# stdstu12/YUME

Measured on AMD Instinct MI355X. Metric: denoise-steps/sec (Yume-5B 720P, 33-frame latent), higher is better.
Workload: dtype bf16; 1 GPU; Yume-5B-720P random-init, 33-frame 704x1280 clip (latent 48x13x44x80, FramePack lfz=8, L=9460), ODE Euler steps of a 50-step shift-7 schedule, no CFG, one chain per GPU; num_layers=30, parallelism=dp1 (independent chains, replicated weights)

## Files before the change

include/yume_hip.h:

```cpp
#ifndef YUME_HIP_H
#define YUME_HIP_H

#include <stdint.h>

#ifdef __cplusplus
extern "C" {
#endif

#define YUME_OK 0
#define YUME_EINVAL (-1)
#define YUME_ELAUNCH (-2)
#define YUME_EUNSUP (-3)

const char* yume_last_error(void);
#define YUME_ABI_VERSION 9
int yume_abi_version(void);
const char* yume_target_arch(void);

int64_t yume_counter_workspace_bytes(void);
int yume_counter_workspace_init(void* ptr, int64_t bytes, void* stream);

int yume_calibrate_mfma(int64_t iters, int64_t workgroups, void* ticks, void* sink, void* stream);

int yume_adaln_modulate(const float* x, int64_t ldx, int64_t T, int64_t C, float eps,
                        const float* mul, const float* add, int64_t tab_stride,
                        const int32_t* row_idx, int add_one,
                        void* out, int64_t ldo, int out_kind, void* stream);

enum {
    YUME_EPI_BF16 = 0,
    YUME_EPI_BF16_GELU = 1,
    YUME_EPI_F32 = 2,
    YUME_EPI_RESID = 3,
    YUME_EPI_BF16_SPLITT = 4,
    YUME_EPI_BF16_GELU_ERF = 5,
    YUME_EPI_BF16_GEGLU = 6
};
int yume_gemm_bf16(const void* A, int64_t lda, const void* W, int64_t ldw, const float* bias,
                   int64_t M, int64_t N, int64_t K, int epi,
                   void* out, int64_t ldo,
                   const float* gate, int64_t gate_stride, const int32_t* row_idx,
                   void* outT, int64_t ldt, int64_t n_split,
                   int variant, void* stream);

int64_t yume_gemm_workspace_bytes(void);
int yume_gemm_bf16_ws(const void* A, int64_t lda, const void* W, int64_t ldw, const float* bias,
                      int64_t M, int64_t N, int64_t K, int epi,
                      void* out, int64_t ldo,
                      const float* gate, int64_t gate_stride, const int32_t* row_idx,
                      void* outT, int64_t ldt, int64_t n_split,
                      int variant, void* workspace, int64_t workspace_bytes, void* stream);

int yume_rmsnorm_rope(void* buf, int64_t ld, int64_t T, int64_t C, int nparts,
                      const float* w, float eps, const float* rope, int64_t D, void* stream);
int yume_rmsnorm_rows_periodic(void* buf, int64_t ld, int64_t T, int64_t C, const float* w, int64_t wperiod, float eps,
                               void* stream);

#define YUME_ATTN_Q_PRESCALED 0x100
#define YUME_ATTN_KV_PADDED 0x200
int yume_attn_fwd(const void* Q, int64_t ldq, const void* K, int64_t ldk, const void* Vt, int64_t ldvt,
                  void* O, int64_t ldo, int64_t Lq, int64_t Lk, int64_t H, float scale,
                  int accumulate, int variant, void* stream);
int64_t yume_attn_workspace_bytes(int64_t Lq, int64_t Lk, int64_t H);
int yume_attn_fwd_ws(const void* Q, int64_t ldq, const void* K, int64_t ldk, const void* Vt, int64_t ldvt,
                     void* O, int64_t ldo, int64_t Lq, int64_t Lk, int64_t H, float scale,
                     int accumulate, int variant, void* workspace, int64_t workspace_bytes, void* stream);
int yume_attn_fwd_kw(const void* Q, int64_t ldq, const void* K, int64_t ldk, const void* Vt, int64_t ldvt,
                     void* O, int64_t ldo, int64_t Lq, int64_t Lk, int64_t H, float scale,
                     int accumulate, int variant, void* workspace, int64_t workspace_bytes, float last_key_weight, void* stream);
int yume_attn_fwd_seg(const void* Q, int64_t ldq, const void* const* K, int64_t ldk, const void* const* Vt, int64_t ldvt,
                      void* O, int64_t ldo, int64_t nseg, int64_t Lq_seg, int64_t seg_pitch, const int64_t* Lk, int64_t H,
                      float scale, int accumulate, int variant, const float* last_key_weight, void* stream);
int64_t yume_attn_batch_workspace_bytes(int64_t nseg, int64_t Lq_seg, int64_t Lk_seg, int64_t H);
int yume_attn_fwd_batch(const void* Q, int64_t ldq, const void* K, int64_t ldk, const void* Vt, int64_t ldvt,
                        void* O, int64_t ldo, int64_t nseg, int64_t Lq_seg, int64_t q_pitch,
                        int64_t Lk_seg, int64_t k_pitch, int64_t H, float scale, int accumulate, int variant,
                        void* workspace, int64_t workspace_bytes, void* stream);

int yume_linear_smallm_f32(const float* in, int64_t R, int64_t K, const void* W, int w_bf16,
                           const float* bias, int64_t N, int in_act, int out_act,
                           const float* add_table, float* out, void* stream);

int yume_sinusoidal_embed(const double* t, const int32_t* t_index, int64_t R, int64_t dim,
                          float* out, void* stream);

int yume_modulation_table(const float* tab, const float* e0, int64_t B, int64_t R, int64_t W,
                          float* out, void* stream);

int yume_patch_gather(const void* x, int in_bf16, int64_t Cin, int64_t F, int64_t H, int64_t W,
                      int64_t f0, int64_t nf, int64_t kh, int64_t kw,
                      void* out, int64_t Kp, void* stream);

int yume_unpatchify(const float* in, int64_t ldi, int64_t Fr, int64_t Hp, int64_t Wp,
                    int64_t ph, int64_t pw, int64_t Cout, float* out, void* stream);

int yume_cast_bf16(const float* in, int64_t ldi, int64_t rows_valid, int64_t rows, int64_t cols,
                   void* out, int64_t ldo, void* stream);
int yume_transpose_bf16(const void* in, int in_bf16, int64_t ldi, int64_t rows, int64_t cols,
                        void* out, int64_t ldo, void* stream);


enum { YUME_CONV_EPI_ADD = 16, YUME_CONV_EPI_TSPLIT = 17, YUME_CONV_EPI_RMS_SILU = 18 };
int yume_conv3d_cl(const void* x, const void* cache, int64_t ldc, int64_t Tin, int64_t Hin, int64_t Win, int64_t Cin,
                   const void* W, int64_t ldw, const float* bias, int64_t Cout,
                   int kt, int kh, int kw, int st, int sh, int sw, int pt, int ph, int pw, int ups,
                   int64_t To, int64_t Ho, int64_t Wo, int epi, void* out, int64_t ldo,
                   const void* add, int64_t ldadd, const void* zero_page, void* stream);

int yume_vae_rmsnorm_silu(const void* x, int64_t ldx, int64_t M, int64_t C, const float* gamma, const float* beta,
                          int silu, void* y, int64_t ldy, void* stream);

int yume_vae_dupup_add(const void* x, int64_t ldx, int64_t Tin, int64_t Hin, int64_t Win, int64_t Cin,
                       void* y, int64_t ldy, int64_t To, int64_t Cout, int ft, int fs, int toff, void* stream);

int yume_vae_avgdown_add(const void* x, int64_t ldx, int64_t Tin, int64_t Hin, int64_t Win, int64_t Cin,
                         void* y, int64_t ldy, int64_t Cout, int ft, int fs, void* stream);

int yume_softmax_rows(const float* S, int64_t lds, int64_t R, int64_t n, float scale, void* P, int64_t ldp, void* stream);

int yume_vae_pack_input(const void* x, int in_bf16, int64_t C, int64_t T, int64_t H, int64_t W, int ps,
                        const float* mul, const float* add, void* out, int64_t Cpad, void* stream);
int yume_vae_unpack_output(const void* x, int64_t ldx, int64_t T, int64_t H, int64_t W, int64_t Cv, int ps,
                           const float* sub, const float* mul, float lo, float hi, float* out, void* stream);

int yume_frames_u8(const float* video, int64_t C, int64_t T, int64_t H, int64_t W, void* out, void* stream);
int yume_frames_u8_trunc(const float* video, int64_t C, int64_t T, int64_t H, int64_t W, void* out, void* stream);

int yume_rmsnorm_f32(const float* x, int64_t ldx, int64_t T, int64_t C, float eps, const float* w, void* out, int64_t ldo,
                     void* stream);
int yume_gemm_bf16_batched(const void* A, int64_t lda, int64_t strideA, const void* W, int64_t ldw, int64_t strideW,
                           int64_t M, int64_t N, int64_t K, int epi, void* out, int64_t ldo, int64_t strideO,
                           int64_t batch, int variant, void* stream);
int yume_softmax_bias_rows(const float* S, int64_t lds, int64_t strideS, int64_t H, int64_t n, const float* bias,
                           int64_t ldb, void* P, int64_t ldp, int64_t strideP, void* stream);
int64_t yume_gemm_splitk_workspace_bytes(int64_t M, int64_t N, int splits);
int yume_gemm_bf16_splitk(const void* A, int64_t lda, const void* W, int64_t ldw, const float* bias, int64_t M, int64_t N,
                          int64_t K, int epi, void* out, int64_t ldo, int splits, void* workspace, void* stream);

#ifdef __cplusplus
}
#endif
#endif
```

yume_amd/_lib.py:

```python
import ctypes
import os
from ctypes import c_void_p, c_int, c_int64, c_float, c_char_p

_HERE = os.path.dirname(os.path.abspath(__file__))
LIB_PATH = os.environ.get("YUME_HIP_LIB") or os.path.join(_HERE, "lib", "libyume_hip.so")

_P, _I, _L, _F = c_void_p, c_int, c_int64, c_float

SIGNATURES = {
    "yume_last_error": [],
    "yume_abi_version": [],
    "yume_target_arch": [],
    "yume_counter_workspace_bytes": [],
    "yume_counter_workspace_init": [_P, _L, _P],
    "yume_calibrate_mfma": [_L, _L, _P, _P, _P],
    "yume_adaln_modulate": [_P, _L, _L, _L, _F, _P, _P, _L, _P, _I, _P, _L, _I, _P],
    "yume_gemm_bf16": [_P, _L, _P, _L, _P, _L, _L, _L, _I, _P, _L, _P, _L, _P, _P, _L, _L, _I, _P],
    "yume_gemm_workspace_bytes": [],
    "yume_gemm_bf16_ws": [_P, _L, _P, _L, _P, _L, _L, _L, _I, _P, _L, _P, _L, _P, _P, _L, _L, _I, _P, _L, _P],
    "yume_rmsnorm_f32": [_P, _L, _L, _L, _F, _P, _P, _L, _P],
    "yume_gemm_bf16_batched": [_P, _L, _L, _P, _L, _L, _L, _L, _L, _I, _P, _L, _L, _L, _I, _P],
    "yume_gemm_splitk_workspace_bytes": [_L, _L, _I],
    "yume_gemm_bf16_splitk": [_P, _L, _P, _L, _P, _L, _L, _L, _I, _P, _L, _I, _P, _P],
    "yume_softmax_bias_rows": [_P, _L, _L, _L, _L, _P, _L, _P, _L, _L, _P],
    "yume_rmsnorm_rows_periodic": [_P, _L, _L, _L, _P, _L, _F, _P],
    "yume_rmsnorm_rope": [_P, _L, _L, _L, _I, _P, _F, _P, _L, _P],
    "yume_attn_fwd": [_P, _L, _P, _L, _P, _L, _P, _L, _L, _L, _L, _F, _I, _I, _P],
    "yume_attn_workspace_bytes": [_L, _L, _L],
    "yume_attn_fwd_ws": [_P, _L, _P, _L, _P, _L, _P, _L, _L, _L, _L, _F, _I, _I, _P, _L, _P],
    "yume_attn_fwd_kw": [_P, _L, _P, _L, _P, _L, _P, _L, _L, _L, _L, _F, _I, _I, _P, _L, _F, _P],
    "yume_attn_fwd_seg": [_P, _L, _P, _L, _P, _L, _P, _L, _L, _L, _L, _P, _L, _F, _I, _I, _P, _P],
    "yume_attn_batch_workspace_bytes": [_L, _L, _L, _L],
    "yume_attn_fwd_batch": [_P, _L, _P, _L, _P, _L, _P, _L, _L, _L, _L, _L, _L, _L, _F, _I, _I, _P, _L, _P],
    "yume_linear_smallm_f32": [_P, _L, _L, _P, _I, _P, _L, _I, _I, _P, _P, _P],
    "yume_sinusoidal_embed": [_P, _P, _L, _L, _P, _P],
    "yume_modulation_table": [_P, _P, _L, _L, _L, _P, _P],
    "yume_patch_gather": [_P, _I, _L, _L, _L, _L, _L, _L, _L, _L, _P, _L, _P],
    "yume_unpatchify": [_P, _L, _L, _L, _L, _L, _L, _L, _P, _P],
    "yume_cast_bf16": [_P, _L, _L, _L, _L, _P, _L, _P],
    "yume_transpose_bf16": [_P, _I, _L, _L, _L, _P, _L, _P],
    "yume_conv3d_cl": [_P, _P, _L, _L, _L, _L, _L, _P, _L, _P, _L, _I, _I, _I, _I, _I, _I, _I, _I, _I, _I, _L, _L, _L, _I, _P, _L,
                       _P, _L, _P, _P],
    "yume_vae_rmsnorm_silu": [_P, _L, _L, _L, _P, _P, _I, _P, _L, _P],
    "yume_vae_dupup_add": [_P, _L, _L, _L, _L, _L, _P, _L, _L, _L, _I, _I, _I, _P],
    "yume_vae_avgdown_add": [_P, _L, _L, _L, _L, _L, _P, _L, _L, _I, _I, _P],
    "yume_softmax_rows": [_P, _L, _L, _L, _F, _P, _L, _P],
    "yume_vae_pack_input": [_P, _I, _L, _L, _L, _L, _I, _P, _P, _P, _L, _P],
    "yume_frames_u8": [_P, _L, _L, _L, _L, _P, _P],
    "yume_frames_u8_trunc": [_P, _L, _L, _L, _L, _P, _P],
    "yume_vae_unpack_output": [_P, _L, _L, _L, _L, _L, _I, _P, _P, _F, _F, _P, _P],
}
_RES = {"yume_last_error": c_char_p, "yume_target_arch": c_char_p, "yume_gemm_splitk_workspace_bytes": c_int64, "yume_attn_workspace_bytes": c_int64,
        "yume_attn_batch_workspace_bytes": c_int64,
        "yume_counter_workspace_bytes": c_int64, "yume_gemm_workspace_bytes": c_int64}

_lib = None
ABI_VERSION = 9


def load():
    global _lib
    if _lib is not None:
        return _lib
    if not os.path.exists(LIB_PATH):
        raise RuntimeError(
            f"{LIB_PATH} is missing: the HIP extension has not been built. "
            "Run `python -c 'import __graft_entry__ as g; g.build()'` (or `python -m yume_amd.build`). "
            "There is no CPU/PyTorch fallback for the yume_amd hot path.")
    import torch
    lib = ctypes.CDLL(LIB_PATH)
    for name, argtypes in SIGNATURES.items():
        fn = getattr(lib, name)
        fn.argtypes = argtypes
        fn.restype = _RES.get(name, c_int)
    got, arch = int(lib.yume_abi_version()), lib.yume_target_arch()
    if got != ABI_VERSION or arch != b"gfx950":
        raise RuntimeError(f"{LIB_PATH} has ABI version {got} for {arch!r}, this binding needs {ABI_VERSION} for gfx950: "
                           "rebuild with `python -m yume_amd.build --force`")
    _lib = lib
    return lib


def check(rc, what):
    if rc != 0:
        msg = load().yume_last_error()
        raise RuntimeError(f"{what} failed (rc={rc}): {msg.decode() if msg else '?'}")
```

yume_amd/csrc/gemm_bf16.hip:

```cpp
#include "gemm_core.hpp"
#include "gemm_w4.hpp"

using namespace gemm_core;

namespace {
bool w4_auto() {
    static const bool on = [] { const char* v = getenv("YUME_GEMM_W4"); return !v || atoi(v) != 0; }();
    return on;
}
bool gemm_log() {
    static const bool on = [] { const char* v = getenv("YUME_GEMM_LOG"); return v && atoi(v) != 0; }();
    return on;
}
void gemm_log_line(const char* kernel, int64_t M, int64_t N, int64_t K, int epi, int variant, int64_t lda, int64_t ldw, int64_t ldo, int64_t ldt,
                   int64_t n_split, bool ws, int64_t batch) {
    fprintf(stderr, "[gemm_bf16] %s M=%lld N=%lld K=%lld epi=%d variant=%d lda=%lld ldw=%lld ldo=%lld ldt=%lld n_split=%lld ws=%d batch=%lld\n", kernel,
            (long long)M, (long long)N, (long long)K, epi, variant, (long long)lda, (long long)ldw, (long long)ldo, (long long)ldt, (long long)n_split,
            ws ? 1 : 0, (long long)batch);
}
}

extern "C" int64_t yume_gemm_workspace_bytes(void) { return gemm_w4::sk_workspace_bytes(gemm_w4::SK_MAX_SLOTS); }

extern "C" int yume_gemm_bf16(const void* A, int64_t lda, const void* W, int64_t ldw, const float* bias, int64_t M,
                              int64_t N, int64_t K, int epi, void* out, int64_t ldo, const float* gate,
                              int64_t gate_stride, const int32_t* row_idx, void* outT, int64_t ldt, int64_t n_split,
                              int variant, void* stream) {
    return yume_gemm_bf16_ws(A, lda, W, ldw, bias, M, N, K, epi, out, ldo, gate, gate_stride, row_idx, outT, ldt, n_split, variant, nullptr, 0, stream);
}

extern "C" int yume_gemm_bf16_ws(const void* A, int64_t lda, const void* W, int64_t ldw, const float* bias, int64_t M,
                                 int64_t N, int64_t K, int epi, void* out, int64_t ldo, const float* gate,
                                 int64_t gate_stride, const int32_t* row_idx, void* outT, int64_t ldt, int64_t n_split,
                                 int variant, void* workspace, int64_t workspace_bytes, void* stream) {
    YUME_REQUIRE(A && W && out, "gemm_bf16: NULL pointer");
    YUME_REQUIRE(M > 0 && N > 0 && K > 0, "gemm_bf16: empty problem M=%lld N=%lld K=%lld", (long long)M, (long long)N, (long long)K);
    YUME_REQUIRE(M < (1ll << 31) && N < (1ll << 31) && K < (1ll << 31), "gemm_bf16: dimension too large");
    YUME_REQUIRE((K % BK) == 0, "gemm_bf16: K=%lld must be a multiple of %d", (long long)K, BK);
    YUME_REQUIRE((N % 4) == 0, "gemm_bf16: N=%lld must be a multiple of 4", (long long)N);
    YUME_REQUIRE((lda % 8) == 0 && (ldw % 8) == 0, "gemm_bf16: lda/ldw must be multiples of 8 (16-byte rows)");
    YUME_REQUIRE((ldo % 4) == 0, "gemm_bf16: ldo must be a multiple of 4");
    YUME_REQUIRE(((uintptr_t)A % 16) == 0 && ((uintptr_t)W % 16) == 0 && ((uintptr_t)out % 16) == 0, "gemm_bf16: pointers must be 16-byte aligned");
    Problem p;
    p.W = (const unsigned short*)W; p.ldw = ldw;
    p.M = (int)M; p.N = (int)N; p.K = (int)K;
    p.tiles_m = (int)((M + BM - 1) / BM);
    p.tiles_n = (int)((N + BN - 1) / BN);
    p.group_m = 8;
    p.bsW = 0; p.bsO = 0;
    bool sk = false;
    if (variant == 0 && workspace != nullptr && w4_auto() && epi != YUME_EPI_BF16_GEGLU &&
        use_256(p, 0, epi != YUME_EPI_BF16_SPLITT || (n_split % 256) == 0) && gemm_w4::w4_applies(p, lda, epi) &&
        (epi != YUME_EPI_BF16_SPLITT || (ldt % 8) == 0)) {
        Problem q = p;
        q.tiles_m = (int)((M + 255) / 256);
        q.tiles_n = (int)((N + 255) / 256);
        gemm_w4::w4_sk_plan(q, workspace, workspace_bytes);
        sk = q.sk_wgs != 0;
    }
    if (!sk && variant == 0 && epi != YUME_EPI_BF16_GEGLU && use_256(p, 0, epi != YUME_EPI_BF16_SPLITT || (n_split % 256) == 0)) {
        const int64_t tn = (N + 255) / 256, tm = (M + 255) / 256, T = tm * tn, R = T % 256, full = T - R;
        const int64_t m_main = full / tn, M_main = m_main * 256, rem = M - M_main;
        if (R > 0 && R <= 96 && full >= 256 && m_main >= 1 && rem > 0 && rem <= 1024) {
            const int64_t osz = (epi == YUME_EPI_F32 || epi == YUME_EPI_RESID) ? 4 : 2;
            auto remainder = [&](void* s2) {
                return yume_gemm_bf16(reinterpret_cast<const unsigned short*>(A) + M_main * lda, lda, W, ldw, bias, rem, N, K, epi,
                                      reinterpret_cast<char*>(out) + M_main * ldo * osz, ldo, gate, gate_stride,
                                      row_idx ? row_idx + M_main : nullptr,
                                      outT ? reinterpret_cast<unsigned short*>(outT) + M_main : nullptr, ldt, n_split, 1, s2);
            };
            int rc = yume_gemm_bf16(A, lda, W, ldw, bias, M_main, N, K, epi, out, ldo, gate, gate_stride, row_idx, outT, ldt, n_split,
                                    w4_auto() ? 3 : 2, stream);
            if (rc != YUME_OK) return rc;
            return remainder(stream);
        }
    }
    PlainA al;
    al.A = (const unsigned short*)A; al.lda = lda; al.M = (int)M; al.bsA = 0;
    Epilogue e = {};
    e.bias = bias;
    e.out = out; e.ldo = ldo;
    e.gate = gate; e.gate_stride = gate_stride; e.row_idx = row_idx;
    e.outT = (unsigned short*)outT; e.ldt = ldt; e.n_split = (int)n_split;
    hipStream_t st = (hipStream_t)stream;
    const bool split_ok = epi != YUME_EPI_BF16_SPLITT || (n_split % 256) == 0;
    const bool big = use_256(p, variant == 3 ? 2 : variant, split_ok);
    const bool w4 = (variant == 3 || (variant == 0 && big && w4_auto())) && split_ok && gemm_w4::w4_applies(p, lda, epi) &&
                    (epi != YUME_EPI_BF16_SPLITT || (ldt % 8) == 0);
    if (gemm_log())
        gemm_log_line(epi == YUME_EPI_BF16_GEGLU ? "g256" : w4 ? (sk ? "w4+sk" : "w4") : big ? "g256" : "g128", M, N, K, epi, variant, lda, ldw, ldo, ldt,
                      n_split, workspace != nullptr, 1);
#define YUME_GO(E) (w4 ? gemm_w4::launch_w4(E, p, al, e, st, "gemm_bf16", variant == 0 ? workspace : nullptr, workspace_bytes) : big ? launch256<E>(p, al, e, st, "gemm_bf16") : launch<E>(p, al, e, st, "gemm_bf16"))
    switch (epi) {
        case YUME_EPI_BF16: return YUME_GO(YUME_EPI_BF16);
        case YUME_EPI_BF16_GELU: return YUME_GO(YUME_EPI_BF16_GELU);
        case YUME_EPI_BF16_GELU_ERF: return YUME_GO(YUME_EPI_BF16_GELU_ERF);
        case YUME_EPI_F32: return YUME_GO(YUME_EPI_F32);
        case YUME_EPI_RESID:
            YUME_REQUIRE(gate == nullptr || (gate_stride % 4) == 0, "gemm_bf16: gate_stride must be a multiple of 4");
            return YUME_GO(YUME_EPI_RESID);
        case YUME_EPI_BF16_GEGLU:
            YUME_REQUIRE((N % 8) == 0 && bias == nullptr, "gemm_bf16: GEGLU needs N %% 8 == 0 and no bias");
            return launch256<YUME_EPI_BF16_GEGLU>(p, al, e, st, "gemm_bf16");
        case YUME_EPI_BF16_SPLITT:
            YUME_REQUIRE(outT != nullptr && n_split >= 0 && (n_split % BN) == 0 && ldt >= M && (ldt % 4) == 0,
                         "gemm_bf16: SPLITT needs outT, n_split %% 128 == 0, ldt >= M and ldt %% 4 == 0");
            YUME_REQUIRE(((uintptr_t)outT % 16) == 0, "gemm_bf16: outT must be 16-byte aligned");
            return YUME_GO(YUME_EPI_BF16_SPLITT);
        default:
            yume_set_error("gemm_bf16: unknown epilogue %d", epi);
            return YUME_EINVAL;
    }
}

extern "C" int yume_gemm_bf16_batched(const void* A, int64_t lda, int64_t strideA, const void* W, int64_t ldw, int64_t strideW,
                                      int64_t M, int64_t N, int64_t K, int epi, void* out, int64_t ldo, int64_t strideO,
                                      int64_t batch, int variant, void* stream) {
    (void)variant;
    YUME_REQUIRE(A && W && out, "gemm_bf16_batched: NULL pointer");
    YUME_REQUIRE(epi == YUME_EPI_BF16 || epi == YUME_EPI_F32, "gemm_bf16_batched: only the plain bf16 / fp32 epilogues");
    YUME_REQUIRE(batch >= 1 && batch <= 65535, "gemm_bf16_batched: batch %lld", (long long)batch);
    YUME_REQUIRE(M > 0 && N > 0 && K > 0 && M < (1ll << 31) && N < (1ll << 31) && K < (1ll << 31), "gemm_bf16_batched: bad problem size");
    YUME_REQUIRE((K % BK) == 0 && (N % 4) == 0, "gemm_bf16_batched: K must be a multiple of %d and N of 4", BK);
    YUME_REQUIRE((lda % 8) == 0 && (ldw % 8) == 0 && (ldo % 4) == 0, "gemm_bf16_batched: lda/ldw must be multiples of 8, ldo of 4");
    YUME_REQUIRE((strideA % 8) == 0 && (strideW % 8) == 0 && (strideO % 8) == 0, "gemm_bf16_batched: strides must keep 16-byte alignment");
    YUME_REQUIRE(((uintptr_t)A % 16) == 0 && ((uintptr_t)W % 16) == 0 && ((uintptr_t)out % 16) == 0, "gemm_bf16_batched: pointers must be 16-byte aligned");
    Problem p;
    p.W = (const unsigned short*)W; p.ldw = ldw;
    p.M = (int)M; p.N = (int)N; p.K = (int)K;
    p.tiles_m = (int)((M + BM - 1) / BM);
    p.tiles_n = (int)((N + BN - 1) / BN);
    p.group_m = 8;
    p.bsW = strideW;
    p.bsO = strideO * (epi == YUME_EPI_F32 ? 4 : 2);
    PlainA al;
    al.A = (const unsigned short*)A; al.lda = lda; al.M = (int)M; al.bsA = strideA;
    Epilogue e = {};
    e.out = out; e.ldo = ldo;
    hipStream_t st = (hipStream_t)stream;
    if (gemm_log()) gemm_log_line("batched", M, N, K, epi, variant, lda, ldw, ldo, 0, 0, false, batch);
    if (epi == YUME_EPI_F32) return launch<YUME_EPI_F32>(p, al, e, st, "gemm_bf16_batched", (int)batch);
    return launch<YUME_EPI_BF16>(p, al, e, st, "gemm_bf16_batched", (int)batch);
}

namespace {
template <int EPI>
__global__ __launch_bounds__(256) void splitk_reduce_kernel(const float* __restrict__ ws, int splits, int64_t MN, int N,
                                                            const float* __restrict__ bias, void* __restrict__ out, int64_t ldo) {
    const int64_t nq = MN >> 2;
    for (int64_t i = (int64_t)blockIdx.x * blockDim.x + threadIdx.x; i < nq; i += (int64_t)gridDim.x * blockDim.x) {
        f32x4 v = *reinterpret_cast<const f32x4*>(ws + 4 * i);
        for (int s = 1; s < splits; ++s) v += *reinterpret_cast<const f32x4*>(ws + s * MN + 4 * i);
        const int64_t m = (4 * i) / N;
        const int n = (int)((4 * i) - m * N);
        if (bias) v += *reinterpret_cast<const f32x4*>(bias + n);
        if (EPI == YUME_EPI_F32) {
            *reinterpret_cast<f32x4*>(reinterpret_cast<float*>(out) + m * ldo + n) = v;
        } else if (EPI == YUME_EPI_RESID) {
            float* xo = reinterpret_cast<float*>(out) + m * ldo + n;
            *reinterpret_cast<f32x4*>(xo) = *reinterpret_cast<const f32x4*>(xo) + v;
        } else if (EPI == YUME_EPI_BF16_GEGLU) {
            const unsigned o = pack_bf16x2(v[1] * gelu_tanh(v[0]), v[3] * gelu_tanh(v[2]));
            *reinterpret_cast<unsigned*>(reinterpret_cast<unsigned short*>(out) + m * ldo + (n >> 1)) = o;
        } else {
            if (EPI == YUME_EPI_BF16_GELU) {
#pragma unroll
                for (int q = 0; q < 4; ++q) v[q] = gelu_tanh(v[q]);
            }
            if (EPI == YUME_EPI_BF16_GELU_ERF) {
#pragma unroll
                for (int q = 0; q < 4; ++q) v[q] = 0.5f * v[q] * (1.0f + erff(v[q] * 0.7071067811865476f));
            }
            u32x2 o;
            o[0] = pack_bf16x2(v[0], v[1]);
            o[1] = pack_bf16x2(v[2], v[3]);
            *reinterpret_cast<u32x2*>(reinterpret_cast<unsigned short*>(out) + m * ldo + n) = o;
        }
    }
}
}

extern "C" int64_t yume_gemm_splitk_workspace_bytes(int64_t M, int64_t N, int splits) { return (int64_t)splits * M * N * 4; }

extern "C" int yume_gemm_bf16_splitk(const void* A, int64_t lda, const void* W, int64_t ldw, const float* bias, int64_t M, int64_t N,
                                     int64_t K, int epi, void* out, int64_t ldo, int splits, void* workspace, void* stream) {
    YUME_REQUIRE(A && W && out && workspace, "gemm_bf16_splitk: NULL pointer");
    YUME_REQUIRE(splits >= 1 && splits <= 64 && (K % (splits * BK)) == 0, "gemm_bf16_splitk: K=%lld must be a multiple of splits*%d (splits=%d)",
                 (long long)K, BK, splits);
    YUME_REQUIRE(M > 0 && N > 0 && (N % 8) == 0 && (ldo % 4) == 0, "gemm_bf16_splitk: N must be a multiple of 8, ldo of 4");
    YUME_REQUIRE(((uintptr_t)workspace % 16) == 0 && ((uintptr_t)out % 16) == 0, "gemm_bf16_splitk: pointers must be 16-byte aligned");
    YUME_REQUIRE((M * N) % 4 == 0, "gemm_bf16_splitk: M*N must be a multiple of 4");
    const int64_t Ks = K / splits;
    int rc = yume_gemm_bf16_batched(A, lda, Ks, W, ldw, Ks, M, N, Ks, YUME_EPI_F32, workspace, N, M * N, splits, 1, stream);
    if (rc != YUME_OK) return rc;
    const int64_t MN = M * N;
    const unsigned grid = (unsigned)((MN / 4 + 255) / 256 > 16384 ? 16384 : (MN / 4 + 255) / 256);
    hipStream_t st = (hipStream_t)stream;
    const float* ws = (const float*)workspace;
    if (gemm_log() && (epi == YUME_EPI_F32 || epi == YUME_EPI_RESID || epi == YUME_EPI_BF16 || epi == YUME_EPI_BF16_GELU || epi == YUME_EPI_BF16_GELU_ERF ||
                       epi == YUME_EPI_BF16_GEGLU))
        gemm_log_line("splitk_reduce", M, N, K, epi, 0, lda, ldw, ldo, 0, 0, true, splits);
#define YUME_RED(E) hipLaunchKernelGGL((splitk_reduce_kernel<E>), dim3(grid), dim3(256), 0, st, ws, splits, MN, (int)N, bias, out, ldo)
    switch (epi) {
        case YUME_EPI_F32: YUME_RED(YUME_EPI_F32); break;
        case YUME_EPI_RESID: YUME_RED(YUME_EPI_RESID); break;
        case YUME_EPI_BF16: YUME_RED(YUME_EPI_BF16); break;
        case YUME_EPI_BF16_GELU: YUME_RED(YUME_EPI_BF16_GELU); break;
        case YUME_EPI_BF16_GELU_ERF: YUME_RED(YUME_EPI_BF16_GELU_ERF); break;
        case YUME_EPI_BF16_GEGLU: YUME_RED(YUME_EPI_BF16_GEGLU); break;
        default:
            yume_set_error("gemm_bf16_splitk: unsupported epilogue %d", epi);
            return YUME_EINVAL;
    }
    YUME_CHECK_LAUNCH("gemm_bf16_splitk");
    return YUME_OK;
}
```

yume_amd/csrc/gemm_w4.hpp:

```cpp
#pragma once
#include "gemm_core.hpp"
#include "trace.hpp"

namespace gemm_w4 {
using namespace gemm_core;

constexpr int NTHR_W4 = 256;
constexpr int OPER_BYTES = 256 * 128;
constexpr int BUF_BYTES = 2 * OPER_BYTES;
constexpr int LDS_W4 = 2 * BUF_BYTES;

#define W4_AG8(n) "a" #n "0", "a" #n "1", "a" #n "2", "a" #n "3", "a" #n "4", "a" #n "5", "a" #n "6", "a" #n "7", "a" #n "8", "a" #n "9"
#define W4_AGPRS "a0", "a1", "a2", "a3", "a4", "a5", "a6", "a7", "a8", "a9", W4_AG8(1), W4_AG8(2), W4_AG8(3), W4_AG8(4), W4_AG8(5), W4_AG8(6), \
    W4_AG8(7), W4_AG8(8), W4_AG8(9), W4_AG8(10), W4_AG8(11), W4_AG8(12), W4_AG8(13), W4_AG8(14), W4_AG8(15), W4_AG8(16), W4_AG8(17), W4_AG8(18), \
    W4_AG8(19), W4_AG8(20), W4_AG8(21), W4_AG8(22), W4_AG8(23), W4_AG8(24), "a250", "a251", "a252", "a253", "a254", "a255"

#define W4_MFMA2(T0, X0, Y0, T1, X1, Y1)                                                                                                         \
    asm volatile("v_mfma_f32_16x16x32_bf16 a[%c4:%c5], %0, %1, a[%c4:%c5]\n\tv_mfma_f32_16x16x32_bf16 a[%c6:%c7], %2, %3, a[%c6:%c7]"             \
                 ::"v"(X0), "v"(Y0), "v"(X1), "v"(Y1), "n"((T0) * 4), "n"((T0) * 4 + 3), "n"((T1) * 4), "n"((T1) * 4 + 3) : "memory", W4_AGPRS)
#define W4_MFMA2_DMA(T0, X0, Y0, T1, X1, Y1, voff, sbase, lbase, loff)                                                                            \
    asm volatile("s_add_u32 m0, %10, %11\n\tv_mfma_f32_16x16x32_bf16 a[%c4:%c5], %0, %1, a[%c4:%c5]\n\tglobal_load_lds_dwordx4 %8, %9\n\t"         \
                 "v_mfma_f32_16x16x32_bf16 a[%c6:%c7], %2, %3, a[%c6:%c7]"                                                                       \
                 ::"v"(X0), "v"(Y0), "v"(X1), "v"(Y1), "n"((T0) * 4), "n"((T0) * 4 + 3), "n"((T1) * 4), "n"((T1) * 4 + 3), "v"(voff), "s"(sbase),   \
                 "s"(lbase), "n"(loff) : "memory", "scc", W4_AGPRS)
#define W4_MFMA2_DMAB(T0, X0, Y0, T1, X1, Y1, voff, srd, soff, lbase, loff)                                                                           \
    asm volatile("s_add_u32 m0, %11, %12\n\tv_mfma_f32_16x16x32_bf16 a[%c4:%c5], %0, %1, a[%c4:%c5]\n\tbuffer_load_dwordx4 %8, %9, %10 offen lds\n\t"  \
                 "v_mfma_f32_16x16x32_bf16 a[%c6:%c7], %2, %3, a[%c6:%c7]"                                                                           \
                 ::"v"(X0), "v"(Y0), "v"(X1), "v"(Y1), "n"((T0) * 4), "n"((T0) * 4 + 3), "n"((T1) * 4), "n"((T1) * 4 + 3), "v"(voff), "s"(srd),         \
                 "s"(soff), "s"(lbase), "n"(loff) : "memory", "scc", W4_AGPRS)
#define W4_DMAB(voff, srd, soff, lbase, loff) \
    asm volatile("s_add_u32 m0, %3, %4\n\ts_nop 0\n\tbuffer_load_dwordx4 %0, %1, %2 offen lds" ::"v"(voff), "s"(srd), "s"(soff), "s"(lbase), "n"(loff) : "memory", "scc")
#define W4_DMA(voff, sbase, lbase, loff) \
    asm volatile("s_add_u32 m0, %2, %3\n\ts_nop 0\n\tglobal_load_lds_dwordx4 %0, %1" ::"v"(voff), "s"(sbase), "s"(lbase), "n"(loff) : "memory", "scc")

template <int R>
__device__ __forceinline__ f32x4 acc_tile() {
    f32x4 v;
    asm volatile("v_accvgpr_read_b32 %0, a[%c4]\n\tv_accvgpr_read_b32 %1, a[%c5]\n\tv_accvgpr_read_b32 %2, a[%c6]\n\tv_accvgpr_read_b32 %3, a[%c7]"
                 : "=v"(v[0]), "=v"(v[1]), "=v"(v[2]), "=v"(v[3]) : "n"(R * 4), "n"(R * 4 + 1), "n"(R * 4 + 2), "n"(R * 4 + 3) : W4_AGPRS);
    return v;
}
template <int R>
__device__ __forceinline__ void acc_tile_add(f32x4 d) {
    f32x4 v = acc_tile<R>();
    v += d;
    asm volatile("v_accvgpr_write_b32 a[%c4], %0\n\tv_accvgpr_write_b32 a[%c5], %1\n\tv_accvgpr_write_b32 a[%c6], %2\n\tv_accvgpr_write_b32 a[%c7], %3"
                 ::"v"(v[0]), "v"(v[1]), "v"(v[2]), "v"(v[3]), "n"(R * 4), "n"(R * 4 + 1), "n"(R * 4 + 2), "n"(R * 4 + 3) : W4_AGPRS);
}
template <int R0, int N>
__device__ __forceinline__ void acc_zero() {
    if constexpr (N > 0) {
        asm volatile("v_accvgpr_write_b32 a[%c0], 0\n\tv_accvgpr_write_b32 a[%c1], 0\n\tv_accvgpr_write_b32 a[%c2], 0\n\tv_accvgpr_write_b32 a[%c3], 0"
                     ::"n"(R0), "n"(R0 + 1), "n"(R0 + 2), "n"(R0 + 3) : W4_AGPRS);
        acc_zero<R0 + 4, N - 4>();
    }
}
template <int I0, int N, typename F>
__device__ __forceinline__ void static_for(F&& f) {
    if constexpr (N > 0) {
        f(std::integral_constant<int, I0>{});
        static_for<I0 + 1, N - 1>(f);
    }
}

struct Ctx {
    char* smem;
    bf16x8_t fa[2][8], fb[2][8];
    unsigned ra1, rb1, ra0n, rb0n;
    unsigned va[8], vb[8];
    const char* pa;
    const char* pb;
    unsigned lcur;
    i32x4 srd;
    unsigned soff, tapmask;
    unsigned mask[8];
    unsigned par[8];
    unsigned uh[2], uw[2];
};

__device__ __forceinline__ bf16x8_t w4_frag(const Ctx& c, unsigned off) { return *reinterpret_cast<const bf16x8_t*>(c.smem + off); }

#define W4_PIECE_LOFF(q) (((q) >> 3) * OPER_BYTES + ((q) & 7) * 4096)

#define W4_X(g) (SWAP ? c.fb[(g) >> 6][(g) & 7] : c.fa[(g) >> 6][((g) & 63) >> 3])
#define W4_Y(g) (SWAP ? c.fa[(g) >> 6][((g) & 63) >> 3] : c.fb[(g) >> 6][(g) & 7])
#define W4_PAIR(g) W4_MFMA2((g) & 63, W4_X(g), W4_Y(g), ((g) + 1) & 63, W4_X((g) + 1), W4_Y((g) + 1))
#define W4_PAIR_DMA(g, voff, sbase, loff) \
    W4_MFMA2_DMA((g) & 63, W4_X(g), W4_Y(g), ((g) + 1) & 63, W4_X((g) + 1), W4_Y((g) + 1), voff, sbase, c.lcur, loff)
#define W4_PAIR_DMAB(g, voff, loff) \
    W4_MFMA2_DMAB((g) & 63, W4_X(g), W4_Y(g), ((g) + 1) & 63, W4_X((g) + 1), W4_Y((g) + 1), voff, c.srd, c.soff, c.lcur, loff)

#ifndef W4_PLAN
#define W4_PLAN 1
#endif
#ifndef W4_ABLATE
#define W4_ABLATE 0
#endif
#ifndef W4_BAR_B
#define W4_BAR_B 35
#endif
#ifndef W4_BAR_A
#define W4_BAR_A 17
#endif
#ifndef W4_DMA0
#define W4_DMA0 (W4_BAR_A + 2)
#endif
constexpr int P_BAR_A = W4_BAR_A;
constexpr int P_BAR_B = W4_BAR_B;
constexpr int dma_pos(int q) { return W4_PLAN == 0 ? W4_DMA0 + q : W4_DMA0 + (q * (63 - W4_DMA0)) / 15; }
constexpr int piece_at(int pos) {
    for (int q = 0; q < 16; ++q)
        if (dma_pos(q) == pos) return q;
    return -1;
}
constexpr int pieces_before_bar_b() {
    int k = 0;
    for (int q = 0; q < 16; ++q) k += dma_pos(q) <= P_BAR_B ? 1 : 0;
    return k;
}
constexpr int P_F0_FIRST = P_BAR_B + 2;
static_assert(P_F0_FIRST + 16 <= 64 && dma_pos(15) <= 63 && 15 < P_BAR_A && dma_pos(0) > P_BAR_A, "the plan must fit the 64 slots");

template <int CONV>
__device__ __forceinline__ unsigned w4_conv_voff(const Ctx& c, int q) {
    unsigned v = c.va[q];
    if constexpr (CONV == 2) v += ((c.par[q] & 1u) ? c.uh[1] : c.uh[0]) + ((c.par[q] & 2u) ? c.uw[1] : c.uw[0]);
    return (c.mask[q] & c.tapmask) ? v : 0xffffffffu;
}

template <int g, bool DMA, bool SWAP, int CONV>
__device__ __forceinline__ void w4_gaps(Ctx& c) {
    if constexpr (g < 128) {
        {
            constexpr int k = g >> 1, pos = k;
            constexpr int q = (DMA && !(W4_ABLATE & 1)) ? piece_at(pos) : -1;
            if constexpr (q >= 0 && q < 8) {
                if constexpr (CONV != 0) W4_PAIR_DMAB(g, w4_conv_voff<CONV>(c, q & 7), W4_PIECE_LOFF(q & 15));
                else W4_PAIR_DMA(g, c.va[q & 7], c.pa, W4_PIECE_LOFF(q & 15));
            } else if constexpr (q >= 8) W4_PAIR_DMA(g, c.vb[q & 7], c.pb, W4_PIECE_LOFF(q & 15));
            else W4_PAIR(g);
            if constexpr (pos >= 0 && pos < 16 && !(W4_ABLATE & 2)) {
                if constexpr (pos < 8) c.fb[1][pos & 7] = w4_frag(c, c.rb1 + (pos & 7) * 2048);
                else c.fa[1][pos & 7] = w4_frag(c, c.ra1 + (pos & 7) * 2048);
            }
            if constexpr (k == P_BAR_A) {
                if constexpr ((W4_ABLATE & 20) == 20) asm volatile("" ::: "memory");
                else if constexpr (W4_ABLATE & 16) asm volatile("s_barrier" ::: "memory");
                else if constexpr (W4_ABLATE & 4) asm volatile("s_waitcnt lgkmcnt(0)" ::: "memory");
                else asm volatile("s_waitcnt lgkmcnt(0)\n\ts_barrier" ::: "memory");
            }
            if constexpr (k == P_BAR_B) {
                constexpr int keep = (DMA && !(W4_ABLATE & 1)) ? pieces_before_bar_b() : 0;
                if constexpr ((W4_ABLATE & 12) == 12) asm volatile("" ::: "memory");
                else if constexpr (W4_ABLATE & 8) asm volatile("s_barrier" ::: "memory");
                else if constexpr (W4_ABLATE & 4) asm volatile("s_waitcnt vmcnt(%c0)" ::"n"(keep) : "memory");
                else asm volatile("s_waitcnt vmcnt(%c0)\n\ts_barrier" ::"n"(keep) : "memory");
            }
            if constexpr (pos >= P_F0_FIRST && pos < P_F0_FIRST + 16 && !(W4_ABLATE & 2)) {
                constexpr int r = pos - P_F0_FIRST;
                if constexpr (r < 8) c.fb[0][r & 7] = w4_frag(c, c.rb0n + (r & 7) * 2048);
                else c.fa[0][r & 7] = w4_frag(c, c.ra0n + (r & 7) * 2048);
            }
            w4_gaps<g + 2, DMA, SWAP, CONV>(c);
        }
    }
}
template <int q, int CONV>
__device__ __forceinline__ void w4_stage_all(Ctx& c) {
    if constexpr (q < 16) {
        if constexpr (q < 8) {
            if constexpr (CONV != 0) W4_DMAB(w4_conv_voff<CONV>(c, q & 7), c.srd, c.soff, c.lcur, W4_PIECE_LOFF(q));
            else W4_DMA(c.va[q & 7], c.pa, c.lcur, W4_PIECE_LOFF(q));
        } else W4_DMA(c.vb[q & 7], c.pb, c.lcur, W4_PIECE_LOFF(q));
        w4_stage_all<q + 1, CONV>(c);
    }
}

template <int EPI>
__device__ __forceinline__ f32x4 w4_act(f32x4 v) {
    if (EPI == YUME_EPI_BF16_GELU) {
        const f32x2_t lo = gelu_tanh2(f32x2_t{v[0], v[1]}), hi = gelu_tanh2(f32x2_t{v[2], v[3]});
        v = f32x4{lo[0], lo[1], hi[0], hi[1]};
    }
    if (EPI == YUME_EPI_BF16_GELU_ERF) {
#pragma unroll
        for (int q = 0; q < 4; ++q) v[q] = 0.5f * v[q] * (1.0f + erff(v[q] * 0.7071067811865476f));
    }
    return v;
}

__device__ __forceinline__ void w4_store_image(char* smem, unsigned short* dst, int64_t ld, int row0, int rows_valid, int col0, int cols_valid) {
    const int lane = threadIdx.x & 63;
    const int wave = __builtin_amdgcn_readfirstlane(threadIdx.x >> 6);
    const int l31 = lane & 31, rh = lane >> 5;
    if (cols_valid == 256) {
        const unsigned lrow = (unsigned)((wave * 64 + rh) * 512), lch = (unsigned)((l31 ^ rh) << 4);
        char* o = reinterpret_cast<char*>(dst + col0 + l31 * 8) + (int64_t)(row0 + wave * 64 + rh) * ld * 2;
        const int64_t step = ld * 4;
        const int rleft = rows_valid - wave * 64 - rh;
        auto rows = [&](auto pred) {
            constexpr bool PRED = decltype(pred)::value;
#pragma unroll
            for (int g = 0; g < 4; ++g) {
                u32x4 d[8];
#pragma unroll
                for (int u = 0; u < 8; ++u) {
                    const int it = g * 8 + u;
                    d[u] = *reinterpret_cast<const u32x4*>(smem + lrow + it * 1024 + (lch ^ (unsigned)(32 * (it & 15))));
                }
#pragma unroll
                for (int u = 0; u < 8; ++u) {
                    const int it = g * 8 + u;
                    if (!PRED || 2 * it < rleft) *reinterpret_cast<u32x4*>(o + it * step) = d[u];
                }
            }
        };
        if (rows_valid == 256) rows(std::false_type{});
        else rows(std::true_type{});
        return;
    }
    unsigned short* out = dst + col0 + l31 * 8;
    const int col_left = cols_valid - l31 * 8;
#pragma unroll 2
    for (int it = 0; it < 32; ++it) {
        const int r = wave * 64 + it * 2 + rh;
        const u32x4 d = *reinterpret_cast<const u32x4*>(smem + r * 512 + (((l31 ^ r) & 31) << 4));
        if (r < rows_valid && col_left > 0) {
            unsigned short* o = out + (int64_t)(row0 + r) * ld;
            if (col_left >= 8) {
                *reinterpret_cast<u32x4*>(o) = d;
            } else {
#pragma unroll
                for (int q = 0; q < 7; ++q)
                    if (q < col_left) o[q] = (unsigned short)(d[q >> 1] >> (16 * (q & 1)));
            }
        }
    }
}

struct ImageOff { unsigned e[8], o[8]; };
__device__ __forceinline__ ImageOff w4_image_offsets(int rsel, int csel, int l15, int l4) {
    ImageOff r;
    const unsigned base = (unsigned)((rsel * 128 + l15) * 512 + (l4 & 1) * 8), ux = (unsigned)(((l4 >> 1) ^ l15) << 4);
#pragma unroll
    for (int b = 0; b < 8; ++b) {
        const unsigned ob = (unsigned)(32 * b) ^ ux;
        r.e[b] = base + 256u * (unsigned)csel + ob;
        r.o[b] = base + 256u * (unsigned)(csel ^ 1) + ob;
    }
    return r;
}

template <int EPI, bool SWAP>
__device__ __forceinline__ void w4_epilogue(const Problem& p, const Epilogue& e, int m0, int n0, char* smem) {
    const int lane = threadIdx.x & 63;
    const int wave = __builtin_amdgcn_readfirstlane(threadIdx.x >> 6);
    const int wr = wave >> 1, wc = wave & 1;
    const int l15 = lane & 15, l4 = lane >> 4;
    constexpr bool BF16_OUT = EPI == YUME_EPI_BF16 || EPI == YUME_EPI_BF16_GELU || EPI == YUME_EPI_BF16_GELU_ERF || EPI == YUME_EPI_BF16_SPLITT ||
                              EPI == EPI_BF16_ADD || EPI == EPI_BF16_TSPLIT;
    if constexpr (!SWAP) {
        float bn[8];
#pragma unroll
        for (int j = 0; j < 8; ++j) bn[j] = e.bias ? e.bias[min(n0 + wc * 128 + 16 * j + l15, p.N - 1)] : 0.f;
        const ImageOff io = w4_image_offsets(wc, wr, l15, l4);
        asm volatile("s_waitcnt lgkmcnt(0)\n\ts_barrier" ::: "memory");
        static_for<0, 64>([&](auto tt) {
            constexpr int T = decltype(tt)::value, i = T >> 3, j = T & 7;
            const f32x4 v = acc_tile<T>();
            u32x2 o;
            o[0] = pack_bf16x2(v[0] + bn[j], v[1] + bn[j]);
            o[1] = pack_bf16x2(v[2] + bn[j], v[3] + bn[j]);
            *reinterpret_cast<u32x2*>(smem + ((j & 1) ? io.o[i] : io.e[i]) + j * 8192) = o;
        });
        asm volatile("s_waitcnt lgkmcnt(0)\n\ts_barrier" ::: "memory");
        w4_store_image(smem, e.outT + (int64_t)(n0 - e.n_split) * e.ldt, e.ldt, 0, min(256, p.N - n0), m0, min(256, p.M - m0));
        return;
    } else {
        if (BF16_OUT && !p.epi_direct && (e.ldo % 8) == 0) {
            f32x4 b[8];
            if (n0 + 256 <= p.N) {
#pragma unroll
                for (int j = 0; j < 8; ++j)
                    b[j] = e.bias ? *reinterpret_cast<const f32x4*>(e.bias + n0 + wc * 128 + 16 * j + 4 * l4) : f32x4{0.f, 0.f, 0.f, 0.f};
            } else {
#pragma unroll
                for (int j = 0; j < 8; ++j) {
                    const int n = n0 + wc * 128 + 16 * j + 4 * l4;
                    b[j] = (e.bias && n + 3 < p.N) ? *reinterpret_cast<const f32x4*>(e.bias + n) : f32x4{0.f, 0.f, 0.f, 0.f};
                }
            }
            const ImageOff io = w4_image_offsets(wr, wc, l15, l4);
            asm volatile("s_waitcnt lgkmcnt(0)\n\ts_barrier" ::: "memory");
            TRACE_STAMP(3);
            static_for<0, 8>([&](auto ii) {
                constexpr int i = decltype(ii)::value;
                u32x2 a2[8];
                if constexpr (EPI == EPI_BF16_ADD) {
                    const int r = wr * 128 + 16 * i + l15;
                    const int nl = n0 + wc * 128 + 4 * l4;
                    const unsigned short* ap = e.add + (int64_t)min(m0 + r, p.M - 1) * e.ldadd + nl;
#pragma unroll
                    for (int j = 0; j < 8; ++j)
                        a2[j] = nl + 16 * j + 3 < p.N ? *reinterpret_cast<const u32x2*>(ap + 16 * j) : u32x2{0u, 0u};
                }
                static_for<0, 8>([&](auto jj) {
                    constexpr int j = decltype(jj)::value;
                    f32x4 v = w4_act<EPI>(acc_tile<i * 8 + j>() + b[j]);
                    if constexpr (EPI == EPI_BF16_ADD) {
                        v[0] += bf16_to_f32((unsigned short)(a2[j][0] & 0xffffu));
                        v[1] += bf16_to_f32((unsigned short)(a2[j][0] >> 16));
                        v[2] += bf16_to_f32((unsigned short)(a2[j][1] & 0xffffu));
                        v[3] += bf16_to_f32((unsigned short)(a2[j][1] >> 16));
                    }
                    u32x2 o;
                    o[0] = pack_bf16x2(v[0], v[1]);
                    o[1] = pack_bf16x2(v[2], v[3]);
                    *reinterpret_cast<u32x2*>(smem + ((i & 1) ? io.o[j] : io.e[j]) + i * 8192) = o;
                });
            });
            asm volatile("s_waitcnt lgkmcnt(0)\n\ts_barrier" ::: "memory");
            TRACE_STAMP(4);
            if constexpr (EPI == EPI_BF16_TSPLIT) {
                const int ch = p.N >> 1, jh = n0 >= ch ? 1 : 0, t = m0 / e.hw;
                w4_store_image(smem, reinterpret_cast<unsigned short*>(e.out), e.ldo, m0 + (t + jh) * e.hw, min(256, p.M - m0), n0 - jh * ch, 256);
            } else {
                w4_store_image(smem, reinterpret_cast<unsigned short*>(e.out), e.ldo, m0, min(256, p.M - m0), n0, min(256, p.N - n0));
            }
            return;
        }
        if (EPI == YUME_EPI_RESID && n0 + 256 <= p.N) {
            f32x4 b[8];
#pragma unroll
            for (int j = 0; j < 8; ++j)
                b[j] = e.bias ? *reinterpret_cast<const f32x4*>(e.bias + n0 + wc * 128 + 16 * j + 4 * l4) : f32x4{0.f, 0.f, 0.f, 0.f};
            const int mrow = m0 + wr * 128 + l15, ncol = n0 + wc * 128 + 4 * l4;
            const bool ragged_m = m0 + 256 > p.M;
            const int mlast = p.M - 1 - mrow;
            float* const xo = reinterpret_cast<float*>(e.out) + (int64_t)mrow * e.ldo + ncol;
            const int64_t xstep = 16 * e.ldo;
            auto xoff = [&](int i) -> int64_t { return ragged_m ? (int64_t)(min(16 * i, mlast) ) * e.ldo : i * xstep; };
            const bool gated = e.gate != nullptr;
            bool rowed = gated && e.row_idx != nullptr;
            int ridx[8];
#pragma unroll
            for (int i = 0; i < 8; ++i) ridx[i] = rowed ? e.row_idx[min(mrow + 16 * i, p.M - 1)] : 0;
            f32x4 x[2][8], g[2][8];
            auto issue_x = [&](auto ii, auto bb) {
                constexpr int i = decltype(ii)::value, bf = decltype(bb)::value;
#pragma unroll
                for (int j = 0; j < 8; ++j) x[bf][j] = *reinterpret_cast<const f32x4*>(xo + xoff(i) + 16 * j);
            };
            auto issue_g = [&](auto ii, auto bb) {
                constexpr int i = decltype(ii)::value, bf = decltype(bb)::value;
                if (rowed || (gated && i < 2)) {
                    const float* gp = e.gate + (int64_t)ridx[i] * e.gate_stride + ncol;
#pragma unroll
                    for (int j = 0; j < 8; ++j) g[bf][j] = *reinterpret_cast<const f32x4*>(gp + 16 * j);
                }
            };
            issue_x(std::integral_constant<int, 0>{}, std::integral_constant<int, 0>{});
            issue_x(std::integral_constant<int, 1>{}, std::integral_constant<int, 1>{});
            if (rowed) {
                const int r0 = __builtin_amdgcn_readfirstlane(ridx[0]);
                bool same = true;
#pragma unroll
                for (int i = 0; i < 8; ++i) same &= ridx[i] == r0;
                if (__all(same)) rowed = false;
            }
            issue_g(std::integral_constant<int, 0>{}, std::integral_constant<int, 0>{});
            issue_g(std::integral_constant<int, 1>{}, std::integral_constant<int, 1>{});
            TRACE_STAMP(3);
            static_for<0, 8>([&](auto ii) {
                constexpr int i = decltype(ii)::value, bf = i & 1;
                static_for<0, 8>([&](auto jj) {
                    constexpr int j = decltype(jj)::value;
                    const f32x4 v = acc_tile<i * 8 + j>() + b[j];
                    if (gated) x[bf][j] += v * g[bf][j];
                    else x[bf][j] += v;
                    if (!ragged_m || 16 * i <= mlast) *reinterpret_cast<f32x4*>(xo + i * xstep + 16 * j) = x[bf][j];
                });
                if constexpr (i + 2 < 8) {
                    issue_x(std::integral_constant<int, i + 2>{}, std::integral_constant<int, bf>{});
                    issue_g(std::integral_constant<int, i + 2>{}, std::integral_constant<int, bf>{});
                }
                if (i == 0) TRACE_STAMP(4);
            });
            TRACE_STAMP(5);
#ifdef YUME_TRACE
            asm volatile("s_waitcnt vmcnt(0)" ::: "memory");
            TRACE_STAMP(6);
#endif
            return;
        }
        static_for<0, 64>([&](auto tt) {
            constexpr int T = decltype(tt)::value, i = T >> 3, j = T & 7;
            const f32x4 v = acc_tile<T>();
            const int m = m0 + wr * 128 + 16 * i + l15, n = n0 + wc * 128 + 16 * j + 4 * l4;
            if (m < p.M && n < p.N) store_row4<EPI>(v, m, n, p, e);
        });
    }
}

template <bool DMA, bool SWAP>
__device__ __forceinline__ void w4_loop(Ctx& c, int t0, int t1, unsigned lbase) {
    for (int t = t0; t < t1; ++t) {
        w4_gaps<0, DMA, SWAP, 0>(c);
        if constexpr (DMA) {
            c.pa += 128;
            c.pb += 128;
        }
        c.lcur = lbase + (((t + 1) & 1) ? BUF_BYTES : 0);
        c.ra1 ^= BUF_BYTES;
        c.rb1 ^= BUF_BYTES;
        c.ra0n ^= BUF_BYTES;
        c.rb0n ^= BUF_BYTES;
    }
}

template <bool SWAP>
__device__ __forceinline__ void w4_mainloop(const Problem& p, const PlainA& al, char* smem, int m0, int n0, int kt0, int nk) {
    const int tid = threadIdx.x;
    const int lane = tid & 63;
    const int wave = __builtin_amdgcn_readfirstlane(tid >> 6);
    const int wr = wave >> 1, wc = wave & 1;
    Ctx c;
    c.smem = smem;
    const unsigned lbase = (unsigned)(uintptr_t)(__attribute__((address_space(3))) char*)smem + wave * 1024;
    c.lcur = lbase;
    c.pa = reinterpret_cast<const char*>(al.A + (int64_t)m0 * al.lda) + (int64_t)kt0 * 128;
    c.pb = reinterpret_cast<const char*>(p.W + (int64_t)n0 * p.ldw) + (int64_t)kt0 * 128;
    const unsigned lda_b = (unsigned)al.lda * 2u, ldw_b = (unsigned)p.ldw * 2u;
    {
        const int rl = 8 * wave + (lane >> 3);
        const unsigned ch = (unsigned)(((lane & 7) ^ (rl & 7)) << 4);
        const int mleft = p.M - 1 - m0, nleft = p.N - 1 - n0;
#pragma unroll
        for (int j = 0; j < 8; ++j) {
            const int r = 32 * j + rl;
            c.va[j] = (unsigned)min(r, mleft) * lda_b + ch;
            c.vb[j] = (unsigned)min(r, nleft) * ldw_b + ch;
        }
    }
    const unsigned sw0 = (unsigned)(((lane >> 4) ^ (lane & 7)) << 4), sw1 = (unsigned)(((4 | (lane >> 4)) ^ (lane & 7)) << 4);
    const unsigned rowa = wr * 16384 + (lane & 15) * 128, rowb = OPER_BYTES + wc * 16384 + (lane & 15) * 128;
    w4_stage_all<0, 0>(c);
    c.pa += 128;
    c.pb += 128;
    c.lcur = lbase + BUF_BYTES;
    w4_stage_all<0, 0>(c);
    c.pa += 128;
    c.pb += 128;
    c.lcur = lbase;
    acc_zero<0, 256>();
    asm volatile("s_waitcnt vmcnt(16)\n\ts_barrier" ::: "memory");
#pragma unroll
    for (int r = 0; r < 8; ++r) {
        c.fb[0][r] = w4_frag(c, rowb + sw0 + r * 2048);
        c.fa[0][r] = w4_frag(c, rowa + sw0 + r * 2048);
    }
    c.ra1 = rowa + sw1;
    c.rb1 = rowb + sw1;
    c.ra0n = BUF_BYTES + rowa + sw0;
    c.rb0n = BUF_BYTES + rowb + sw0;
    w4_loop<true, SWAP>(c, 0, nk - 2, lbase);
    w4_loop<false, SWAP>(c, nk - 2, nk, lbase);
    asm volatile("s_waitcnt lgkmcnt(0)\n\ts_barrier" ::: "memory");
    asm volatile("s_nop 15\n\ts_nop 15" ::: "memory");
}

constexpr int SK_SLOT_BYTES = 64 * NTHR_W4 * 16;
constexpr int SK_FLAG_STRIDE = 64;
constexpr int SK_MIN_KT = 4;
constexpr int SK_MAX_SLOTS = 256;
constexpr unsigned SK_SPIN_LIMIT = 1u << 22;

__host__ __device__ __forceinline__ int64_t sk_workspace_bytes(int slots) { return (int64_t)slots * (SK_SLOT_BYTES + SK_FLAG_STRIDE) + 64; }

template <int T0, int N>
__device__ __forceinline__ void sk_publish_tiles(const char* slot, unsigned lane_off) {
    if constexpr (N > 0) {
        const f32x4 v = acc_tile<T0>();
        asm volatile("global_store_dwordx4 %0, %1, %2 sc1\n\ts_nop 1" ::"v"(lane_off + (unsigned)(T0 * (NTHR_W4 * 16))), "v"(v), "s"(slot) : "memory");
        sk_publish_tiles<T0 + 1, N - 1>(slot, lane_off);
    }
}
template <int T0, int N>
__device__ __forceinline__ void sk_gather_tiles(const char* slot, unsigned lane_off) {
    if constexpr (N > 0) {
        f32x4 d[8];
#pragma unroll
        for (int u = 0; u < 8; ++u) d[u] = *reinterpret_cast<const f32x4*>(slot + (lane_off + (unsigned)((T0 + u) * (NTHR_W4 * 16))));
        static_for<0, 8>([&](auto uu) {
            constexpr int u = decltype(uu)::value;
            acc_tile_add<T0 + u>(d[u]);
        });
        sk_gather_tiles<T0 + 8, N - 8>(slot, lane_off);
    }
}

template <bool SWAP>
__device__ __forceinline__ void w4_finish_piece(const Problem& p, const Epilogue& e, int epi, char* smem, int m0, int n0, int slot, int t, int nslice) {
    typedef unsigned gu32;
    char* const slots = p.sk_ws;
    gu32* const flags = reinterpret_cast<gu32*>(p.sk_ws + (int64_t)SK_MAX_SLOTS * SK_SLOT_BYTES);
    unsigned lane_off = threadIdx.x * 16u;
    asm volatile("" : "+v"(lane_off));
    if (slot >= 0) {
        sk_publish_tiles<0, 64>(slots + (int64_t)slot * SK_SLOT_BYTES, lane_off);
        asm volatile("s_waitcnt vmcnt(0)" ::: "memory");
        __syncthreads();
        if (threadIdx.x == 0) __hip_atomic_store(flags + slot * (SK_FLAG_STRIDE / 4), 1u, __ATOMIC_RELAXED, __HIP_MEMORY_SCOPE_AGENT);
        return;
    }
    if (nslice > 1) {
        for (int j = 1; j < nslice; ++j) {
            const int q = (j - 1) * p.sk_tiles + t;
            if (threadIdx.x == 0) {
                gu32* f = flags + q * (SK_FLAG_STRIDE / 4);
                unsigned spins = 0;
                while (__hip_atomic_load(f, __ATOMIC_RELAXED, __HIP_MEMORY_SCOPE_AGENT) == 0u) {
                    __builtin_amdgcn_s_sleep(8);
                    if (++spins > SK_SPIN_LIMIT) {
                        __hip_atomic_store(flags + SK_MAX_SLOTS * (SK_FLAG_STRIDE / 4), 1u, __ATOMIC_RELAXED, __HIP_MEMORY_SCOPE_AGENT);
                        break;
                    }
                }
                __builtin_amdgcn_fence(__ATOMIC_ACQUIRE, "agent");
                asm volatile("s_waitcnt vmcnt(0)" ::: "memory");
            }
            __syncthreads();
            sk_gather_tiles<0, 64>(slots + (int64_t)q * SK_SLOT_BYTES, lane_off);
            __syncthreads();
            if (threadIdx.x == 0) __hip_atomic_store(flags + q * (SK_FLAG_STRIDE / 4), 0u, __ATOMIC_RELAXED, __HIP_MEMORY_SCOPE_AGENT);
        }
        asm volatile("s_nop 15" ::: "memory");
    }
    TRACE_STAMP(1);
    if constexpr (!SWAP) {
        w4_epilogue<YUME_EPI_BF16_SPLITT, false>(p, e, m0, n0, smem);
    } else {
        switch (epi) {
#ifndef W4_EXPERIMENT
            case YUME_EPI_BF16_GELU: w4_epilogue<YUME_EPI_BF16_GELU, true>(p, e, m0, n0, smem); break;
            case YUME_EPI_BF16_GELU_ERF: w4_epilogue<YUME_EPI_BF16_GELU_ERF, true>(p, e, m0, n0, smem); break;
            case YUME_EPI_F32: w4_epilogue<YUME_EPI_F32, true>(p, e, m0, n0, smem); break;
            case YUME_EPI_RESID: w4_epilogue<YUME_EPI_RESID, true>(p, e, m0, n0, smem); break;
            case YUME_EPI_BF16_SPLITT: w4_epilogue<YUME_EPI_BF16_SPLITT, true>(p, e, m0, n0, smem); break;
#endif
            default: w4_epilogue<YUME_EPI_BF16, true>(p, e, m0, n0, smem); break;
        }
    }
}

template <int UNUSED = 0>
__global__ __launch_bounds__(NTHR_W4, 1) void gemm_w4_kernel(Problem p, PlainA al, Epilogue e, int epi) {
    __shared__ __attribute__((aligned(16))) char smem[LDS_W4];
    TRACE_STAMP(0);
    const int nk = p.K / BK;
    const int ndp = p.sk_wgs ? p.sk_dp : p.tiles_m * p.tiles_n;
    int pc0 = 0, pc1 = 1, R = 1, tile0, head_t = 0;
    bool tails = false;
    if ((int)blockIdx.x < ndp) {
        int start, count;
        xcd_chunk(ndp, blockIdx.x & 7, start, count);
        tile0 = start + (blockIdx.x >> 3);
    } else {
        const int sk = (int)blockIdx.x - ndp, per = p.sk_wgs >> 3;
        const int w = (sk & 7) * per + (sk >> 3);
        R = p.sk_tiles;
        tile0 = ndp;
        if (w < R) {
            head_t = w;
        } else {
            tails = true;
            const int ntail = (p.sk_s - 1) * R;
            pc0 = (w - R) * p.sk_q;
            pc1 = min(ntail, pc0 + p.sk_q);
            if (pc0 >= pc1) return;
        }
    }
    for (int pc = pc0; pc < pc1; ++pc) {
        int t = head_t, j = 0, k0 = 0, k1 = nk, slot = -1, nslice = 1;
        if (p.sk_wgs && (int)blockIdx.x >= ndp) {
            if (tails) {
                j = 1 + pc / R;
                t = pc - (j - 1) * R;
                k0 = p.sk_lh + (j - 1) * p.sk_lt;
                k1 = j == p.sk_s - 1 ? nk : k0 + p.sk_lt;
                slot = pc;
            } else {
                k1 = p.sk_lh;
                nslice = p.sk_s;
            }
        }
        int m0, n0;
        tile_origin(p, tile0 + t, m0, n0);
        if (epi == YUME_EPI_BF16_SPLITT && n0 >= e.n_split) {
            w4_mainloop<false>(p, al, smem, m0, n0, k0, k1 - k0);
            w4_finish_piece<false>(p, e, epi, smem, m0, n0, slot, t, nslice);
        } else {
            w4_mainloop<true>(p, al, smem, m0, n0, k0, k1 - k0);
            w4_finish_piece<true>(p, e, epi, smem, m0, n0, slot, t, nslice);
        }
        if (pc + 1 < pc1) __syncthreads();
    }
    TRACE_STAMP(2);
}

inline bool w4_applies(const Problem& p, int64_t lda, int epi) {
    if (p.K < 3 * BK) return false;
#ifdef W4_EXPERIMENT
    if (epi != YUME_EPI_BF16) return false;
#endif
    if (255ll * lda * 2 + 128 >= (1ll << 32) || 255ll * p.ldw * 2 + 128 >= (1ll << 32)) return false;
    return epi == YUME_EPI_BF16 || epi == YUME_EPI_BF16_GELU || epi == YUME_EPI_BF16_GELU_ERF || epi == YUME_EPI_F32 || epi == YUME_EPI_RESID ||
           epi == YUME_EPI_BF16_SPLITT;
}

inline void w4_sk_plan(Problem& p, void* ws, int64_t ws_bytes) {
    p.sk_dp = 0; p.sk_tiles = 0; p.sk_wgs = 0; p.sk_s = 1; p.sk_q = 1; p.sk_lh = 0; p.sk_lt = 0; p.sk_ws = nullptr;
    static const bool on = [] { const char* v = getenv("YUME_GEMM_SK"); return !v || atoi(v) != 0; }();
    static const int ncu = [] {
        int d = 0, n = 0;
        if (hipGetDevice(&d) != hipSuccess || hipDeviceGetAttribute(&n, hipDeviceAttributeMultiprocessorCount, d) != hipSuccess) n = 0;
        return n;
    }();
    if (!on || ws == nullptr || ncu < 64 || ncu > SK_MAX_SLOTS || (ncu & 7) != 0) return;
    if (ws_bytes < sk_workspace_bytes(SK_MAX_SLOTS) || ((uintptr_t)ws & 15) != 0) return;
    const int T = p.tiles_m * p.tiles_n, nk = p.K / BK;
    const int R = T % ncu;
    if (R == 0 || T < ncu) return;
    static const int min_nk = [] { const char* v = getenv("YUME_GEMM_SK_MIN_NK"); return v ? atoi(v) : 96; }();
    if (nk < min_nk) return;
    int s, q, lh, lt;
    if (2 * R > ncu) {
        s = 2;
        q = (R + (ncu - R) - 1) / (ncu - R);
        lt = nk / (q + 1);
        lh = nk - lt;
    } else {
        s = ncu / R;
        if (s > nk / SK_MIN_KT) s = nk / SK_MIN_KT;
        q = 1;
        lt = nk / s;
        lh = lt;
    }
    if (s < 2 || lt < SK_MIN_KT || lh < SK_MIN_KT || (s - 1) * R > SK_MAX_SLOTS) return;
    const int nwg = R + ((s - 1) * R + q - 1) / q;
    if (nwg > ncu) return;
    p.sk_tiles = R;
    p.sk_dp = T - R;
    p.sk_s = s; p.sk_q = q; p.sk_lh = lh; p.sk_lt = lt;
    p.sk_wgs = (nwg + 7) / 8 * 8;
    p.sk_ws = (char*)ws;
}

inline int launch_w4(int epi, const Problem& p128, const PlainA& al, const Epilogue& e, hipStream_t st, const char* what, void* ws = nullptr,
                     int64_t ws_bytes = 0) {
    Problem p = p128;
    p.tiles_m = (p.M + 255) / 256;
    p.tiles_n = (p.N + 255) / 256;
    p.group_m = g_group_m;
    { static const int d = [] { const char* v = getenv("YUME_GEMM_EPI_DIRECT"); return v ? atoi(v) : 0; }(); p.epi_direct = d; }
    w4_sk_plan(p, ws, ws_bytes);
    const unsigned grid = p.sk_wgs ? (unsigned)(p.sk_dp + p.sk_wgs) : (unsigned)(p.tiles_m * p.tiles_n);
    hipLaunchKernelGGL(gemm_w4_kernel<0>, dim3(grid), dim3(NTHR_W4), 0, st, p, al, e, epi);
    YUME_CHECK_LAUNCH(what);
    return YUME_OK;
}

}
```

Before: 10.45 denoise-steps/sec.

## Add 256x192 narrow-tile GEMM variant and band planner to balance wave quantization

Adds a w4n GEMM kernel whose waves own 6 W fragments, giving 256x192 tiles, and generalizes the gap/DMA schedule plan over NJ. A cost-model band planner splits M into a leading band run with 256x256 tiles and a trailing band run with 256x192 tiles, choosing the split that minimizes estimated waves across the CU count. It replaces the old row-split remainder path when it predicts a win and is enabled by default. The aim is to cut tail-wave idle CUs in the large GEMMs, at the cost of an extra launch and a less efficient narrow tile whose throughput is estimated by fixed rho constants.

Result: no change. 10.52 denoise-steps/sec (median of 6 runs) (+0.7%).

```diff
diff --git a/include/yume_hip.h b/include/yume_hip.h
--- a/include/yume_hip.h
+++ b/include/yume_hip.h
@@ -50,6 +50,9 @@
                       const float* gate, int64_t gate_stride, const int32_t* row_idx,
                       void* outT, int64_t ldt, int64_t n_split,
                       int variant, void* workspace, int64_t workspace_bytes, void* stream);
+
+int yume_gemm_band_plan(int64_t M, int64_t N, int64_t K, int epi, int64_t lda, int64_t ldw, int64_t ldt, int64_t n_split, int ncu, int sk,
+                        int* x, int* y);
 
 int yume_rmsnorm_rope(void* buf, int64_t ld, int64_t T, int64_t C, int nparts,
                       const float* w, float eps, const float* rope, int64_t D, void* stream);
diff --git a/yume_amd/_lib.py b/yume_amd/_lib.py
--- a/yume_amd/_lib.py
+++ b/yume_amd/_lib.py
@@ -17,6 +17,7 @@
     "yume_adaln_modulate": [_P, _L, _L, _L, _F, _P, _P, _L, _P, _I, _P, _L, _I, _P],
     "yume_gemm_bf16": [_P, _L, _P, _L, _P, _L, _L, _L, _I, _P, _L, _P, _L, _P, _P, _L, _L, _I, _P],
     "yume_gemm_workspace_bytes": [],
+    "yume_gemm_band_plan": [_L, _L, _L, _I, _L, _L, _L, _L, _I, _I, _P, _P],
     "yume_gemm_bf16_ws": [_P, _L, _P, _L, _P, _L, _L, _L, _I, _P, _L, _P, _L, _P, _P, _L, _L, _I, _P, _L, _P],
     "yume_rmsnorm_f32": [_P, _L, _L, _L, _F, _P, _P, _L, _P],
     "yume_gemm_bf16_batched": [_P, _L, _L, _P, _L, _L, _L, _L, _L, _I, _P, _L, _L, _L, _I, _P],
diff --git a/yume_amd/csrc/gemm_bf16.hip b/yume_amd/csrc/gemm_bf16.hip
--- a/yume_amd/csrc/gemm_bf16.hip
+++ b/yume_amd/csrc/gemm_bf16.hip
@@ -11,6 +11,31 @@
 bool gemm_log() {
     static const bool on = [] { const char* v = getenv("YUME_GEMM_LOG"); return v && atoi(v) != 0; }();
     return on;
+}
+bool band_on() {
+    static const bool on = [] { const char* v = getenv("YUME_GEMM_BAND"); return !v || atoi(v) != 0; }();
+    return on;
+}
+int device_cus() {
+    static const int ncu = [] {
+        int d = 0, n = 0;
+        if (hipGetDevice(&d) != hipSuccess || hipDeviceGetAttribute(&n, hipDeviceAttributeMultiprocessorCount, d) != hipSuccess) n = 0;
+        return n;
+    }();
+    return ncu;
+}
+int64_t row_split_rows(int64_t M, int64_t N) {
+    const int64_t tn = (N + 255) / 256, tm = (M + 255) / 256, T = tm * tn, R = T % 256, full = T - R;
+    const int64_t m_main = full / tn, rem = M - m_main * 256;
+    return (R > 0 && R <= 96 && full >= 256 && m_main >= 1 && rem > 0 && rem <= 1024) ? m_main * 256 : 0;
+}
+int band_route(int64_t M, int64_t N, int64_t K, int epi, int64_t lda, int64_t ldw, int64_t ldt, int64_t n_split, int ncu, bool sk, int* y) {
+    *y = 0;
+    Problem p;
+    p.M = (int)M; p.N = (int)N; p.K = (int)K; p.ldw = ldw;
+    if (epi == YUME_EPI_BF16_GEGLU || !use_256(p, 0, epi != YUME_EPI_BF16_SPLITT || (n_split % 256) == 0)) return -1;
+    if (!gemm_w4::w4n_applies(p, lda, epi, n_split, ldt) || (epi == YUME_EPI_BF16_SPLITT && (ldt % 8) != 0)) return -1;
+    return gemm_w4::w4_band_plan(M, N, K, epi, ncu, sk, row_split_rows(M, N) != 0, y);
 }
 void gemm_log_line(const char* kernel, int64_t M, int64_t N, int64_t K, int epi, int variant, int64_t lda, int64_t ldw, int64_t ldo, int64_t ldt,
                    int64_t n_split, bool ws, int64_t batch) {
@@ -18,6 +43,15 @@
             (long long)M, (long long)N, (long long)K, epi, variant, (long long)lda, (long long)ldw, (long long)ldo, (long long)ldt, (long long)n_split,
             ws ? 1 : 0, (long long)batch);
 }
+}
+
+extern "C" int yume_gemm_band_plan(int64_t M, int64_t N, int64_t K, int epi, int64_t lda, int64_t ldw, int64_t ldt, int64_t n_split, int ncu,
+                                   int sk, int* x, int* y) {
+    int yy = 0;
+    const int xx = band_route(M, N, K, epi, lda, ldw, ldt, n_split, ncu, sk != 0, &yy);
+    if (x) *x = xx < 0 ? 0 : xx;
+    if (y) *y = yy;
+    return xx >= 0 ? 1 : 0;
 }
 
 extern "C" int64_t yume_gemm_workspace_bytes(void) { return gemm_w4::sk_workspace_bytes(gemm_w4::SK_MAX_SLOTS); }
@@ -59,16 +93,28 @@
         sk = q.sk_wgs != 0;
     }
     if (!sk && variant == 0 && epi != YUME_EPI_BF16_GEGLU && use_256(p, 0, epi != YUME_EPI_BF16_SPLITT || (n_split % 256) == 0)) {
-        const int64_t tn = (N + 255) / 256, tm = (M + 255) / 256, T = tm * tn, R = T % 256, full = T - R;
-        const int64_t m_main = full / tn, M_main = m_main * 256, rem = M - M_main;
-        if (R > 0 && R <= 96 && full >= 256 && m_main >= 1 && rem > 0 && rem <= 1024) {
-            const int64_t osz = (epi == YUME_EPI_F32 || epi == YUME_EPI_RESID) ? 4 : 2;
-            auto remainder = [&](void* s2) {
-                return yume_gemm_bf16(reinterpret_cast<const unsigned short*>(A) + M_main * lda, lda, W, ldw, bias, rem, N, K, epi,
-                                      reinterpret_cast<char*>(out) + M_main * ldo * osz, ldo, gate, gate_stride,
-                                      row_idx ? row_idx + M_main : nullptr,
-                                      outT ? reinterpret_cast<unsigned short*>(outT) + M_main : nullptr, ldt, n_split, 1, s2);
-            };
+        const int64_t osz = (epi == YUME_EPI_F32 || epi == YUME_EPI_RESID) ? 4 : 2;
+        auto rows_from = [&](int64_t M0, int var, void* s2) {
+            return yume_gemm_bf16(reinterpret_cast<const unsigned short*>(A) + M0 * lda, lda, W, ldw, bias, M - M0, N, K, epi,
+                                  reinterpret_cast<char*>(out) + M0 * ldo * osz, ldo, gate, gate_stride,
+                                  row_idx ? row_idx + M0 : nullptr,
+                                  outT ? reinterpret_cast<unsigned short*>(outT) + M0 : nullptr, ldt, n_split, var, s2);
+        };
+        if (band_on() && w4_auto()) {
+            int y = 0;
+            const int x = band_route(M, N, K, epi, lda, ldw, ldt, n_split, device_cus(), false, &y);
+            if (x >= 0) {
+                if (x > 0) {
+                    int rc = yume_gemm_bf16(A, lda, W, ldw, bias, (int64_t)x * 256, N, K, epi, out, ldo, gate, gate_stride, row_idx, outT, ldt,
+                                            n_split, 3, stream);
+                    if (rc != YUME_OK) return rc;
+                }
+                return rows_from((int64_t)x * 256, 4, stream);
+            }
+        }
+        const int64_t M_main = row_split_rows(M, N);
+        if (M_main != 0) {
+            auto remainder = [&](void* s2) { return rows_from(M_main, 1, s2); };
             int rc = yume_gemm_bf16(A, lda, W, ldw, bias, M_main, N, K, epi, out, ldo, gate, gate_stride, row_idx, outT, ldt, n_split,
                                     w4_auto() ? 3 : 2, stream);
             if (rc != YUME_OK) return rc;
@@ -83,14 +129,16 @@
     e.gate = gate; e.gate_stride = gate_stride; e.row_idx = row_idx;
     e.outT = (unsigned short*)outT; e.ldt = ldt; e.n_split = (int)n_split;
     hipStream_t st = (hipStream_t)stream;
+    const bool w4n = variant == 4 && gemm_w4::w4n_applies(p, lda, epi, n_split, ldt);
+    if (variant == 4 && !w4n) variant = 3;
     const bool split_ok = epi != YUME_EPI_BF16_SPLITT || (n_split % 256) == 0;
     const bool big = use_256(p, variant == 3 ? 2 : variant, split_ok);
     const bool w4 = (variant == 3 || (variant == 0 && big && w4_auto())) && split_ok && gemm_w4::w4_applies(p, lda, epi) &&
                     (epi != YUME_EPI_BF16_SPLITT || (ldt % 8) == 0);
     if (gemm_log())
-        gemm_log_line(epi == YUME_EPI_BF16_GEGLU ? "g256" : w4 ? (sk ? "w4+sk" : "w4") : big ? "g256" : "g128", M, N, K, epi, variant, lda, ldw, ldo, ldt,
+        gemm_log_line(epi == YUME_EPI_BF16_GEGLU ? "g256" : w4n ? "w4n" : w4 ? (sk ? "w4+sk" : "w4") : big ? "g256" : "g128", M, N, K, epi, variant, lda, ldw, ldo, ldt,
                       n_split, workspace != nullptr, 1);
-#define YUME_GO(E) (w4 ? gemm_w4::launch_w4(E, p, al, e, st, "gemm_bf16", variant == 0 ? workspace : nullptr, workspace_bytes) : big ? launch256<E>(p, al, e, st, "gemm_bf16") : launch<E>(p, al, e, st, "gemm_bf16"))
+#define YUME_GO(E) (w4n ? gemm_w4::launch_w4n(E, p, al, e, st, "gemm_bf16") : w4 ? gemm_w4::launch_w4(E, p, al, e, st, "gemm_bf16", variant == 0 ? workspace : nullptr, workspace_bytes) : big ? launch256<E>(p, al, e, st, "gemm_bf16") : launch<E>(p, al, e, st, "gemm_bf16"))
     switch (epi) {
         case YUME_EPI_BF16: return YUME_GO(YUME_EPI_BF16);
         case YUME_EPI_BF16_GELU: return YUME_GO(YUME_EPI_BF16_GELU);
@@ -103,8 +151,8 @@
             YUME_REQUIRE((N % 8) == 0 && bias == nullptr, "gemm_bf16: GEGLU needs N %% 8 == 0 and no bias");
             return launch256<YUME_EPI_BF16_GEGLU>(p, al, e, st, "gemm_bf16");
         case YUME_EPI_BF16_SPLITT:
-            YUME_REQUIRE(outT != nullptr && n_split >= 0 && (n_split % BN) == 0 && ldt >= M && (ldt % 4) == 0,
-                         "gemm_bf16: SPLITT needs outT, n_split %% 128 == 0, ldt >= M and ldt %% 4 == 0");
+            YUME_REQUIRE(outT != nullptr && n_split >= 0 && ((n_split % BN) == 0 || w4n) && ldt >= M && (ldt % 4) == 0,
+                         "gemm_bf16: SPLITT needs outT, n_split %% 128 == 0 (variant 4: %% 192), ldt >= M and ldt %% 4 == 0");
             YUME_REQUIRE(((uintptr_t)outT % 16) == 0, "gemm_bf16: outT must be 16-byte aligned");
             return YUME_GO(YUME_EPI_BF16_SPLITT);
         default:
diff --git a/yume_amd/csrc/gemm_w4.hpp b/yume_amd/csrc/gemm_w4.hpp
--- a/yume_amd/csrc/gemm_w4.hpp
+++ b/yume_amd/csrc/gemm_w4.hpp
@@ -82,13 +82,17 @@
 
 #define W4_PIECE_LOFF(q) (((q) >> 3) * OPER_BYTES + ((q) & 7) * 4096)
 
-#define W4_X(g) (SWAP ? c.fb[(g) >> 6][(g) & 7] : c.fa[(g) >> 6][((g) & 63) >> 3])
-#define W4_Y(g) (SWAP ? c.fa[(g) >> 6][((g) & 63) >> 3] : c.fb[(g) >> 6][(g) & 7])
-#define W4_PAIR(g) W4_MFMA2((g) & 63, W4_X(g), W4_Y(g), ((g) + 1) & 63, W4_X((g) + 1), W4_Y((g) + 1))
+#define W4_KS(g) ((g) / (8 * NJ))
+#define W4_I(g) (((g) % (8 * NJ)) / NJ)
+#define W4_J(g) (((g) % (8 * NJ)) % NJ)
+#define W4_T(g) (W4_I(g) * 8 + W4_J(g))
+#define W4_X(g) (SWAP ? c.fb[W4_KS(g)][W4_J(g)] : c.fa[W4_KS(g)][W4_I(g)])
+#define W4_Y(g) (SWAP ? c.fa[W4_KS(g)][W4_I(g)] : c.fb[W4_KS(g)][W4_J(g)])
+#define W4_PAIR(g) W4_MFMA2(W4_T(g), W4_X(g), W4_Y(g), W4_T((g) + 1), W4_X((g) + 1), W4_Y((g) + 1))
 #define W4_PAIR_DMA(g, voff, sbase, loff) \
-    W4_MFMA2_DMA((g) & 63, W4_X(g), W4_Y(g), ((g) + 1) & 63, W4_X((g) + 1), W4_Y((g) + 1), voff, sbase, c.lcur, loff)
+    W4_MFMA2_DMA(W4_T(g), W4_X(g), W4_Y(g), W4_T((g) + 1), W4_X((g) + 1), W4_Y((g) + 1), voff, sbase, c.lcur, loff)
 #define W4_PAIR_DMAB(g, voff, loff) \
-    W4_MFMA2_DMAB((g) & 63, W4_X(g), W4_Y(g), ((g) + 1) & 63, W4_X((g) + 1), W4_Y((g) + 1), voff, c.srd, c.soff, c.lcur, loff)
+    W4_MFMA2_DMAB(W4_T(g), W4_X(g), W4_Y(g), W4_T((g) + 1), W4_X((g) + 1), W4_Y((g) + 1), voff, c.srd, c.soff, c.lcur, loff)
 
 #ifndef W4_PLAN
 #define W4_PLAN 1
@@ -105,21 +109,34 @@
 #ifndef W4_DMA0
 #define W4_DMA0 (W4_BAR_A + 2)
 #endif
-constexpr int P_BAR_A = W4_BAR_A;
-constexpr int P_BAR_B = W4_BAR_B;
-constexpr int dma_pos(int q) { return W4_PLAN == 0 ? W4_DMA0 + q : W4_DMA0 + (q * (63 - W4_DMA0)) / 15; }
-constexpr int piece_at(int pos) {
-    for (int q = 0; q < 16; ++q)
-        if (dma_pos(q) == pos) return q;
-    return -1;
-}
-constexpr int pieces_before_bar_b() {
-    int k = 0;
-    for (int q = 0; q < 16; ++q) k += dma_pos(q) <= P_BAR_B ? 1 : 0;
-    return k;
-}
-constexpr int P_F0_FIRST = P_BAR_B + 2;
-static_assert(P_F0_FIRST + 16 <= 64 && dma_pos(15) <= 63 && 15 < P_BAR_A && dma_pos(0) > P_BAR_A, "the plan must fit the 64 slots");
+template <int NJ>
+struct GapPlan {
+    static constexpr int SLOTS = 8 * NJ, NP = 8 + NJ, NR = 8 + NJ;
+    static constexpr int BAR_A = NJ == 8 ? W4_BAR_A : 15;
+    static constexpr int BAR_B = NJ == 8 ? W4_BAR_B : 27;
+    static constexpr int DMA0 = NJ == 8 ? W4_DMA0 : BAR_A + 2;
+    static constexpr int dma_pos(int q) { return W4_PLAN == 0 ? DMA0 + q : DMA0 + (q * (SLOTS - 1 - DMA0)) / (NP - 1); }
+    static constexpr int piece_at(int pos) {
+        for (int q = 0; q < NP; ++q)
+            if (dma_pos(q) == pos) return q;
+        return -1;
+    }
+    static constexpr int pieces_before_bar_b() {
+        int k = 0;
+        for (int q = 0; q < NP; ++q) k += dma_pos(q) <= BAR_B ? 1 : 0;
+        return k;
+    }
+    static constexpr bool pieces_distinct() {
+        for (int q = 1; q < NP; ++q)
+            if (dma_pos(q) <= dma_pos(q - 1)) return false;
+        return true;
+    }
+    static constexpr int F0_FIRST = BAR_B + 2;
+    static_assert(NJ == 8 || NJ == 6, "a wave owns 8 or 6 W fragments");
+    static_assert(F0_FIRST + NR <= SLOTS && dma_pos(NP - 1) <= SLOTS - 1 && NR - 1 < BAR_A && dma_pos(0) > BAR_A && pieces_distinct(),
+                  "the plan must fit the slots");
+    static_assert(BAR_B >= SLOTS / 2, "F0(t+1) overwrites the fragments segment 1 reads: barrier B belongs to segment 2");
+};
 
 template <int CONV>
 __device__ __forceinline__ unsigned w4_conv_voff(const Ctx& c, int q) {
@@ -128,20 +145,22 @@
     return (c.mask[q] & c.tapmask) ? v : 0xffffffffu;
 }
 
-template <int g, bool DMA, bool SWAP, int CONV>
+template <int g, bool DMA, bool SWAP, int CONV, int NJ = 8>
 __device__ __forceinline__ void w4_gaps(Ctx& c) {
-    if constexpr (g < 128) {
+    using P = GapPlan<NJ>;
+    constexpr int P_BAR_A = P::BAR_A, P_BAR_B = P::BAR_B, P_F0_FIRST = P::F0_FIRST;
+    if constexpr (g < 16 * NJ) {
         {
             constexpr int k = g >> 1, pos = k;
-            constexpr int q = (DMA && !(W4_ABLATE & 1)) ? piece_at(pos) : -1;
+            constexpr int q = (DMA && !(W4_ABLATE & 1)) ? P::piece_at(pos) : -1;
             if constexpr (q >= 0 && q < 8) {
                 if constexpr (CONV != 0) W4_PAIR_DMAB(g, w4_conv_voff<CONV>(c, q & 7), W4_PIECE_LOFF(q & 15));
                 else W4_PAIR_DMA(g, c.va[q & 7], c.pa, W4_PIECE_LOFF(q & 15));
             } else if constexpr (q >= 8) W4_PAIR_DMA(g, c.vb[q & 7], c.pb, W4_PIECE_LOFF(q & 15));
             else W4_PAIR(g);
-            if constexpr (pos >= 0 && pos < 16 && !(W4_ABLATE & 2)) {
-                if constexpr (pos < 8) c.fb[1][pos & 7] = w4_frag(c, c.rb1 + (pos & 7) * 2048);
-                else c.fa[1][pos & 7] = w4_frag(c, c.ra1 + (pos & 7) * 2048);
+            if constexpr (pos >= 0 && pos < P::NR && !(W4_ABLATE & 2)) {
+                if constexpr (pos < NJ) c.fb[1][pos] = w4_frag(c, c.rb1 + pos * 2048);
+                else c.fa[1][pos - NJ] = w4_frag(c, c.ra1 + (pos - NJ) * 2048);
             }
             if constexpr (k == P_BAR_A) {
                 if constexpr ((W4_ABLATE & 20) == 20) asm volatile("" ::: "memory");
@@ -150,29 +169,29 @@
                 else asm volatile("s_waitcnt lgkmcnt(0)\n\ts_barrier" ::: "memory");
             }
             if constexpr (k == P_BAR_B) {
-                constexpr int keep = (DMA && !(W4_ABLATE & 1)) ? pieces_before_bar_b() : 0;
+                constexpr int keep = (DMA && !(W4_ABLATE & 1)) ? P::pieces_before_bar_b() : 0;
                 if constexpr ((W4_ABLATE & 12) == 12) asm volatile("" ::: "memory");
                 else if constexpr (W4_ABLATE & 8) asm volatile("s_barrier" ::: "memory");
                 else if constexpr (W4_ABLATE & 4) asm volatile("s_waitcnt vmcnt(%c0)" ::"n"(keep) : "memory");
                 else asm volatile("s_waitcnt vmcnt(%c0)\n\ts_barrier" ::"n"(keep) : "memory");
             }
-            if constexpr (pos >= P_F0_FIRST && pos < P_F0_FIRST + 16 && !(W4_ABLATE & 2)) {
+            if constexpr (pos >= P_F0_FIRST && pos < P_F0_FIRST + P::NR && !(W4_ABLATE & 2)) {
                 constexpr int r = pos - P_F0_FIRST;
-                if constexpr (r < 8) c.fb[0][r & 7] = w4_frag(c, c.rb0n + (r & 7) * 2048);
-                else c.fa[0][r & 7] = w4_frag(c, c.ra0n + (r & 7) * 2048);
-            }
-            w4_gaps<g + 2, DMA, SWAP, CONV>(c);
-        }
-    }
-}
-template <int q, int CONV>
+                if constexpr (r < NJ) c.fb[0][r] = w4_frag(c, c.rb0n + r * 2048);
+                else c.fa[0][r - NJ] = w4_frag(c, c.ra0n + (r - NJ) * 2048);
+            }
+            w4_gaps<g + 2, DMA, SWAP, CONV, NJ>(c);
+        }
+    }
+}
+template <int q, int CONV, int NJ = 8>
 __device__ __forceinline__ void w4_stage_all(Ctx& c) {
-    if constexpr (q < 16) {
+    if constexpr (q < 8 + NJ) {
         if constexpr (q < 8) {
             if constexpr (CONV != 0) W4_DMAB(w4_conv_voff<CONV>(c, q & 7), c.srd, c.soff, c.lcur, W4_PIECE_LOFF(q));
             else W4_DMA(c.va[q & 7], c.pa, c.lcur, W4_PIECE_LOFF(q));
         } else W4_DMA(c.vb[q & 7], c.pb, c.lcur, W4_PIECE_LOFF(q));
-        w4_stage_all<q + 1, CONV>(c);
+        w4_stage_all<q + 1, CONV, NJ>(c);
     }
 }
 
@@ -189,11 +208,12 @@
     return v;
 }
 
+template <int TW = 256, bool A8 = false>
 __device__ __forceinline__ void w4_store_image(char* smem, unsigned short* dst, int64_t ld, int row0, int rows_valid, int col0, int cols_valid) {
     const int lane = threadIdx.x & 63;
     const int wave = __builtin_amdgcn_readfirstlane(threadIdx.x >> 6);
     const int l31 = lane & 31, rh = lane >> 5;
-    if (cols_valid == 256) {
+    if (!A8 && cols_valid == TW) {
         const unsigned lrow = (unsigned)((wave * 64 + rh) * 512), lch = (unsigned)((l31 ^ rh) << 4);
         char* o = reinterpret_cast<char*>(dst + col0 + l31 * 8) + (int64_t)(row0 + wave * 64 + rh) * ld * 2;
         const int64_t step = ld * 4;
@@ -211,7 +231,7 @@
 #pragma unroll
                 for (int u = 0; u < 8; ++u) {
                     const int it = g * 8 + u;
-                    if (!PRED || 2 * it < rleft) *reinterpret_cast<u32x4*>(o + it * step) = d[u];
+                    if ((TW == 256 || l31 < TW / 8) && (!PRED || 2 * it < rleft)) *reinterpret_cast<u32x4*>(o + it * step) = d[u];
                 }
             }
         };
@@ -228,7 +248,12 @@
         if (r < rows_valid && col_left > 0) {
             unsigned short* o = out + (int64_t)(row0 + r) * ld;
             if (col_left >= 8) {
-                *reinterpret_cast<u32x4*>(o) = d;
+                if constexpr (A8) {
+                    *reinterpret_cast<u32x2*>(o) = u32x2{d[0], d[1]};
+                    *reinterpret_cast<u32x2*>(o + 4) = u32x2{d[2], d[3]};
+                } else {
+                    *reinterpret_cast<u32x4*>(o) = d;
+                }
             } else {
 #pragma unroll
                 for (int q = 0; q < 7; ++q)
@@ -251,8 +276,21 @@
     return r;
 }
 
-template <int EPI, bool SWAP>
+__device__ __forceinline__ ImageOff w4_image_offsets_at(int row0, int chunk0, int l15, int l4) {
+    ImageOff r;
+    const unsigned base = (unsigned)((row0 + l15) * 512 + (l4 & 1) * 8);
+#pragma unroll
+    for (int b = 0; b < 8; ++b) {
+        const unsigned ch = (unsigned)(chunk0 + 2 * b + (l4 >> 1));
+        r.e[b] = base + (((ch ^ (unsigned)l15) & 31u) << 4);
+        r.o[b] = base + (((ch ^ (unsigned)(16 + l15)) & 31u) << 4);
+    }
+    return r;
+}
+
+template <int EPI, bool SWAP, int NJ = 8>
 __device__ __forceinline__ void w4_epilogue(const Problem& p, const Epilogue& e, int m0, int n0, char* smem) {
+    constexpr int TW = 32 * NJ, WW = 16 * NJ;
     const int lane = threadIdx.x & 63;
     const int wave = __builtin_amdgcn_readfirstlane(threadIdx.x >> 6);
     const int wr = wave >> 1, wc = wave & 1;
@@ -260,13 +298,13 @@
     constexpr bool BF16_OUT = EPI == YUME_EPI_BF16 || EPI == YUME_EPI_BF16_GELU || EPI == YUME_EPI_BF16_GELU_ERF || EPI == YUME_EPI_BF16_SPLITT ||
                               EPI == EPI_BF16_ADD || EPI == EPI_BF16_TSPLIT;
     if constexpr (!SWAP) {
-        float bn[8];
-#pragma unroll
-        for (int j = 0; j < 8; ++j) bn[j] = e.bias ? e.bias[min(n0 + wc * 128 + 16 * j + l15, p.N - 1)] : 0.f;
-        const ImageOff io = w4_image_offsets(wc, wr, l15, l4);
+        float bn[NJ];
+#pragma unroll
+        for (int j = 0; j < NJ; ++j) bn[j] = e.bias ? e.bias[min(n0 + wc * WW + 16 * j + l15, p.N - 1)] : 0.f;
+        const ImageOff io = NJ == 8 ? w4_image_offsets(wc, wr, l15, l4) : w4_image_offsets_at(wc * WW, wr * 16, l15, l4);
         asm volatile("s_waitcnt lgkmcnt(0)\n\ts_barrier" ::: "memory");
-        static_for<0, 64>([&](auto tt) {
-            constexpr int T = decltype(tt)::value, i = T >> 3, j = T & 7;
+        static_for<0, 8 * NJ>([&](auto tt) {
+            constexpr int i = decltype(tt)::value / NJ, j = decltype(tt)::value % NJ, T = i * 8 + j;
             const f32x4 v = acc_tile<T>();
             u32x2 o;
             o[0] = pack_bf16x2(v[0] + bn[j], v[1] + bn[j]);
@@ -274,37 +312,40 @@
             *reinterpret_cast<u32x2*>(smem + ((j & 1) ? io.o[i] : io.e[i]) + j * 8192) = o;
         });
         asm volatile("s_waitcnt lgkmcnt(0)\n\ts_barrier" ::: "memory");
-        w4_store_image(smem, e.outT + (int64_t)(n0 - e.n_split) * e.ldt, e.ldt, 0, min(256, p.N - n0), m0, min(256, p.M - m0));
+        if (NJ != 8 && (e.ldt % 8) != 0)
+            w4_store_image<256, true>(smem, e.outT + (int64_t)(n0 - e.n_split) * e.ldt, e.ldt, 0, min(TW, p.N - n0), m0, min(256, p.M - m0));
+        else
+            w4_store_image(smem, e.outT + (int64_t)(n0 - e.n_split) * e.ldt, e.ldt, 0, min(TW, p.N - n0), m0, min(256, p.M - m0));
         return;
     } else {
         if (BF16_OUT && !p.epi_direct && (e.ldo % 8) == 0) {
-            f32x4 b[8];
-            if (n0 + 256 <= p.N) {
-#pragma unroll
-                for (int j = 0; j < 8; ++j)
-                    b[j] = e.bias ? *reinterpret_cast<const f32x4*>(e.bias + n0 + wc * 128 + 16 * j + 4 * l4) : f32x4{0.f, 0.f, 0.f, 0.f};
+            f32x4 b[NJ];
+            if (n0 + TW <= p.N) {
+#pragma unroll
+                for (int j = 0; j < NJ; ++j)
+                    b[j] = e.bias ? *reinterpret_cast<const f32x4*>(e.bias + n0 + wc * WW + 16 * j + 4 * l4) : f32x4{0.f, 0.f, 0.f, 0.f};
             } else {
 #pragma unroll
-                for (int j = 0; j < 8; ++j) {
-                    const int n = n0 + wc * 128 + 16 * j + 4 * l4;
+                for (int j = 0; j < NJ; ++j) {
+                    const int n = n0 + wc * WW + 16 * j + 4 * l4;
                     b[j] = (e.bias && n + 3 < p.N) ? *reinterpret_cast<const f32x4*>(e.bias + n) : f32x4{0.f, 0.f, 0.f, 0.f};
                 }
             }
-            const ImageOff io = w4_image_offsets(wr, wc, l15, l4);
+            const ImageOff io = NJ == 8 ? w4_image_offsets(wr, wc, l15, l4) : w4_image_offsets_at(wr * 128, wc * (WW / 8), l15, l4);
             asm volatile("s_waitcnt lgkmcnt(0)\n\ts_barrier" ::: "memory");
             TRACE_STAMP(3);
             static_for<0, 8>([&](auto ii) {
                 constexpr int i = decltype(ii)::value;
-                u32x2 a2[8];
+                u32x2 a2[NJ];
                 if constexpr (EPI == EPI_BF16_ADD) {
                     const int r = wr * 128 + 16 * i + l15;
-                    const int nl = n0 + wc * 128 + 4 * l4;
+                    const int nl = n0 + wc * WW + 4 * l4;
                     const unsigned short* ap = e.add + (int64_t)min(m0 + r, p.M - 1) * e.ldadd + nl;
 #pragma unroll
-                    for (int j = 0; j < 8; ++j)
+                    for (int j = 0; j < NJ; ++j)
                         a2[j] = nl + 16 * j + 3 < p.N ? *reinterpret_cast<const u32x2*>(ap + 16 * j) : u32x2{0u, 0u};
                 }
-                static_for<0, 8>([&](auto jj) {
+                static_for<0, NJ>([&](auto jj) {
                     constexpr int j = decltype(jj)::value;
                     f32x4 v = w4_act<EPI>(acc_tile<i * 8 + j>() + b[j]);
                     if constexpr (EPI == EPI_BF16_ADD) {
@@ -323,18 +364,18 @@
             TRACE_STAMP(4);
             if constexpr (EPI == EPI_BF16_TSPLIT) {
                 const int ch = p.N >> 1, jh = n0 >= ch ? 1 : 0, t = m0 / e.hw;
-                w4_store_image(smem, reinterpret_cast<unsigned short*>(e.out), e.ldo, m0 + (t + jh) * e.hw, min(256, p.M - m0), n0 - jh * ch, 256);
+                w4_store_image<TW>(smem, reinterpret_cast<unsigned short*>(e.out), e.ldo, m0 + (t + jh) * e.hw, min(256, p.M - m0), n0 - jh * ch, TW);
             } else {
-                w4_store_image(smem, reinterpret_cast<unsigned short*>(e.out), e.ldo, m0, min(256, p.M - m0), n0, min(256, p.N - n0));
+                w4_store_image<TW>(smem, reinterpret_cast<unsigned short*>(e.out), e.ldo, m0, min(256, p.M - m0), n0, min(TW, p.N - n0));
             }
             return;
         }
-        if (EPI == YUME_EPI_RESID && n0 + 256 <= p.N) {
-            f32x4 b[8];
-#pragma unroll
-            for (int j = 0; j < 8; ++j)
-                b[j] = e.bias ? *reinterpret_cast<const f32x4*>(e.bias + n0 + wc * 128 + 16 * j + 4 * l4) : f32x4{0.f, 0.f, 0.f, 0.f};
-            const int mrow = m0 + wr * 128 + l15, ncol = n0 + wc * 128 + 4 * l4;
+        if (EPI == YUME_EPI_RESID && n0 + TW <= p.N) {
+            f32x4 b[NJ];
+#pragma unroll
+            for (int j = 0; j < NJ; ++j)
+                b[j] = e.bias ? *reinterpret_cast<const f32x4*>(e.bias + n0 + wc * WW + 16 * j + 4 * l4) : f32x4{0.f, 0.f, 0.f, 0.f};
+            const int mrow = m0 + wr * 128 + l15, ncol = n0 + wc * WW + 4 * l4;
             const bool ragged_m = m0 + 256 > p.M;
             const int mlast = p.M - 1 - mrow;
             float* const xo = reinterpret_cast<float*>(e.out) + (int64_t)mrow * e.ldo + ncol;
@@ -345,18 +386,18 @@
             int ridx[8];
 #pragma unroll
             for (int i = 0; i < 8; ++i) ridx[i] = rowed ? e.row_idx[min(mrow + 16 * i, p.M - 1)] : 0;
-            f32x4 x[2][8], g[2][8];
+            f32x4 x[2][NJ], g[2][NJ];
             auto issue_x = [&](auto ii, auto bb) {
                 constexpr int i = decltype(ii)::value, bf = decltype(bb)::value;
 #pragma unroll
-                for (int j = 0; j < 8; ++j) x[bf][j] = *reinterpret_cast<const f32x4*>(xo + xoff(i) + 16 * j);
+                for (int j = 0; j < NJ; ++j) x[bf][j] = *reinterpret_cast<const f32x4*>(xo + xoff(i) + 16 * j);
             };
             auto issue_g = [&](auto ii, auto bb) {
                 constexpr int i = decltype(ii)::value, bf = decltype(bb)::value;
                 if (rowed || (gated && i < 2)) {
                     const float* gp = e.gate + (int64_t)ridx[i] * e.gate_stride + ncol;
 #pragma unroll
-                    for (int j = 0; j < 8; ++j) g[bf][j] = *reinterpret_cast<const f32x4*>(gp + 16 * j);
+                    for (int j = 0; j < NJ; ++j) g[bf][j] = *reinterpret_cast<const f32x4*>(gp + 16 * j);
                 }
             };
             issue_x(std::integral_constant<int, 0>{}, std::integral_constant<int, 0>{});
@@ -373,7 +414,7 @@
             TRACE_STAMP(3);
             static_for<0, 8>([&](auto ii) {
                 constexpr int i = decltype(ii)::value, bf = i & 1;
-                static_for<0, 8>([&](auto jj) {
+                static_for<0, NJ>([&](auto jj) {
                     constexpr int j = decltype(jj)::value;
                     const f32x4 v = acc_tile<i * 8 + j>() + b[j];
                     if (gated) x[bf][j] += v * g[bf][j];
@@ -393,19 +434,19 @@
 #endif
             return;
         }
-        static_for<0, 64>([&](auto tt) {
-            constexpr int T = decltype(tt)::value, i = T >> 3, j = T & 7;
+        static_for<0, 8 * NJ>([&](auto tt) {
+            constexpr int i = decltype(tt)::value / NJ, j = decltype(tt)::value % NJ, T = i * 8 + j;
             const f32x4 v = acc_tile<T>();
-            const int m = m0 + wr * 128 + 16 * i + l15, n = n0 + wc * 128 + 16 * j + 4 * l4;
+            const int m = m0 + wr * 128 + 16 * i + l15, n = n0 + wc * WW + 16 * j + 4 * l4;
             if (m < p.M && n < p.N) store_row4<EPI>(v, m, n, p, e);
         });
     }
 }
 
-template <bool DMA, bool SWAP>
+template <bool DMA, bool SWAP, int NJ = 8>
 __device__ __forceinline__ void w4_loop(Ctx& c, int t0, int t1, unsigned lbase) {
     for (int t = t0; t < t1; ++t) {
-        w4_gaps<0, DMA, SWAP, 0>(c);
+        w4_gaps<0, DMA, SWAP, 0, NJ>(c);
         if constexpr (DMA) {
             c.pa += 128;
             c.pb += 128;
@@ -418,7 +459,7 @@
     }
 }
 
-template <bool SWAP>
+template <bool SWAP, int NJ = 8>
 __device__ __forceinline__ void w4_mainloop(const Problem& p, const PlainA& al, char* smem, int m0, int n0, int kt0, int nk) {
     const int tid = threadIdx.x;
     const int lane = tid & 63;
@@ -443,28 +484,28 @@
         }
     }
     const unsigned sw0 = (unsigned)(((lane >> 4) ^ (lane & 7)) << 4), sw1 = (unsigned)(((4 | (lane >> 4)) ^ (lane & 7)) << 4);
-    const unsigned rowa = wr * 16384 + (lane & 15) * 128, rowb = OPER_BYTES + wc * 16384 + (lane & 15) * 128;
-    w4_stage_all<0, 0>(c);
+    const unsigned rowa = wr * 16384 + (lane & 15) * 128, rowb = OPER_BYTES + wc * (NJ * 2048) + (lane & 15) * 128;
+    w4_stage_all<0, 0, NJ>(c);
     c.pa += 128;
     c.pb += 128;
     c.lcur = lbase + BUF_BYTES;
-    w4_stage_all<0, 0>(c);
+    w4_stage_all<0, 0, NJ>(c);
     c.pa += 128;
     c.pb += 128;
     c.lcur = lbase;
     acc_zero<0, 256>();
-    asm volatile("s_waitcnt vmcnt(16)\n\ts_barrier" ::: "memory");
+    asm volatile("s_waitcnt vmcnt(%c0)\n\ts_barrier" ::"n"(8 + NJ) : "memory");
 #pragma unroll
     for (int r = 0; r < 8; ++r) {
-        c.fb[0][r] = w4_frag(c, rowb + sw0 + r * 2048);
+        if (r < NJ) c.fb[0][r] = w4_frag(c, rowb + sw0 + r * 2048);
         c.fa[0][r] = w4_frag(c, rowa + sw0 + r * 2048);
     }
     c.ra1 = rowa + sw1;
     c.rb1 = rowb + sw1;
     c.ra0n = BUF_BYTES + rowa + sw0;
     c.rb0n = BUF_BYTES + rowb + sw0;
-    w4_loop<true, SWAP>(c, 0, nk - 2, lbase);
-    w4_loop<false, SWAP>(c, nk - 2, nk, lbase);
+    w4_loop<true, SWAP, NJ>(c, 0, nk - 2, lbase);
+    w4_loop<false, SWAP, NJ>(c, nk - 2, nk, lbase);
     asm volatile("s_waitcnt lgkmcnt(0)\n\ts_barrier" ::: "memory");
     asm volatile("s_nop 15\n\ts_nop 15" ::: "memory");
 }
@@ -670,4 +711,69 @@
     return YUME_OK;
 }
 
-}
+template <int UNUSED = 0>
+__global__ __launch_bounds__(NTHR_W4, 1) void gemm_w4n_kernel(Problem p, PlainA al, Epilogue e, int epi) {
+    __shared__ __attribute__((aligned(16))) char smem[LDS_W4];
+    const int nk = p.K / BK;
+    int start, count, m0, n0;
+    xcd_chunk(p.tiles_m * p.tiles_n, blockIdx.x & 7, start, count);
+    tile_origin(p, start + (blockIdx.x >> 3), m0, n0);
+    n0 = (n0 >> 8) * 192;
+    if (epi == YUME_EPI_BF16_SPLITT && n0 >= e.n_split) {
+        w4_mainloop<false, 6>(p, al, smem, m0, n0, 0, nk);
+        w4_epilogue<YUME_EPI_BF16_SPLITT, false, 6>(p, e, m0, n0, smem);
+    } else {
+        w4_mainloop<true, 6>(p, al, smem, m0, n0, 0, nk);
+        switch (epi) {
+            case YUME_EPI_BF16_GELU: w4_epilogue<YUME_EPI_BF16_GELU, true, 6>(p, e, m0, n0, smem); break;
+            case YUME_EPI_BF16_GELU_ERF: w4_epilogue<YUME_EPI_BF16_GELU_ERF, true, 6>(p, e, m0, n0, smem); break;
+            case YUME_EPI_F32: w4_epilogue<YUME_EPI_F32, true, 6>(p, e, m0, n0, smem); break;
+            case YUME_EPI_RESID: w4_epilogue<YUME_EPI_RESID, true, 6>(p, e, m0, n0, smem); break;
+            case YUME_EPI_BF16_SPLITT: w4_epilogue<YUME_EPI_BF16_SPLITT, true, 6>(p, e, m0, n0, smem); break;
+            default: w4_epilogue<YUME_EPI_BF16, true, 6>(p, e, m0, n0, smem); break;
+        }
+    }
+}
+
+inline bool w4n_applies(const Problem& p, int64_t lda, int epi, int64_t n_split, int64_t ldt) {
+    return w4_applies(p, lda, epi) && (epi != YUME_EPI_BF16_SPLITT || (n_split % 192) == 0);
+}
+
+inline int launch_w4n(int epi, const Problem& p128, const PlainA& al, const Epilogue& e, hipStream_t st, const char* what) {
+    Problem p = p128;
+    p.tiles_m = (p.M + 255) / 256;
+    p.tiles_n = (p.N + 191) / 192;
+    p.group_m = g_group_m;
+    p.epi_direct = 0;
+    p.sk_dp = 0; p.sk_tiles = 0; p.sk_wgs = 0; p.sk_s = 1; p.sk_q = 1; p.sk_lh = 0; p.sk_lt = 0; p.sk_ws = nullptr;
+    hipLaunchKernelGGL(gemm_w4n_kernel<0>, dim3((unsigned)(p.tiles_m * p.tiles_n)), dim3(NTHR_W4), 0, st, p, al, e, epi);
+    YUME_CHECK_LAUNCH(what);
+    return YUME_OK;
+}
+
+constexpr double BAND_RHO_F32 = 0.96;
+constexpr double BAND_RHO_ACT = 0.92;
+constexpr double BAND_RHO_BF16 = 1.04;
+constexpr double BAND_REM_COST = 0.92;
+constexpr double BAND_MARGIN = 0.01;
+constexpr int BAND_MIN_NK = 16;
+
+inline int w4_band_plan(int64_t M, int64_t N, int64_t K, int epi, int ncu, bool sk, bool row_split_ok, int* y_out) {
+    *y_out = 0;
+    if (sk || ncu < 64 || K / BK < BAND_MIN_NK) return -1;
+    const int64_t tm = (M + 255) / 256, tn = (N + 255) / 256, tnn = (N + 191) / 192, T = tm * tn;
+    if (T < ncu || T % ncu == 0) return -1;
+    const double rho = (epi == YUME_EPI_F32 || epi == YUME_EPI_RESID) ? BAND_RHO_F32 : epi == YUME_EPI_BF16 ? BAND_RHO_BF16 : BAND_RHO_ACT;
+    const double today = row_split_ok ? (double)(T / ncu) + BAND_REM_COST : (double)((T + ncu - 1) / ncu);
+    double best = today * (1.0 - BAND_MARGIN);
+    int bx = -1;
+    for (int64_t x = tm - 1; x >= 0; --x) {
+        const double c = (double)((x * tn + ncu - 1) / ncu) + rho * (double)(((tm - x) * tnn + ncu - 1) / ncu);
+        if (c < best) { best = c; bx = (int)x; }
+    }
+    if (bx < 0) return -1;
+    *y_out = (int)(tm - bx);
+    return bx;
+}
+
+}
```
